# gashon/transformer-lm

Measured on AMD Instinct MI355X. Metric: BPE train input MB/s (32k vocab), train_bpe(path) end to end, higher is better.
Workload: dtype int64

## Files before the change

### transformer-lm_amd/csrc/api.hip

```cpp
#include <dlfcn.h>
#include <hip/hip_version.h>

#include <cerrno>
#include <cstdio>
#include <cstdlib>
#include <cstring>
#include <fstream>
#include <memory>
#include <mutex>
#include <string_view>
#include <unordered_map>
#include <unordered_set>
#include <string>
#include <vector>

#include "count.h"
#include "drive.h"
#include "internal.h"

namespace bpe {

namespace {
thread_local std::string g_err;
thread_local int g_errno = 0;
bool g_timing = false;

struct DeviceGuard {
    static void require() {
        int n = 0;
        if (hipGetDeviceCount(&n) != hipSuccess || n == 0)
            throw Error{BPE_E_HIP, "no HIP device visible (libbpe355 needs an MI355X / gfx950 GPU)"};
    }
};

template <class F>
int guarded(F&& f) {
    try {
        f();
        g_err.clear();
        return BPE_OK;
    } catch (const Error& e) {
        g_err = e.msg;
        g_errno = e.sys_errno;
        return e.code;
    } catch (const std::bad_alloc&) {
        g_err = "host allocation failed";
        return BPE_E_NOMEM;
    } catch (const std::exception& e) {
        g_err = e.what();
        return BPE_E_ARG;
    }
}

std::vector<std::string> to_specials(const char* const* specials, int n) {
    BPE_REQUIRE(n >= 0 && (n == 0 || specials), BPE_E_ARG, "bad special token list");
    std::vector<std::string> v;
    for (int i = 0; i < n; ++i) {
        BPE_REQUIRE(specials[i], BPE_E_ARG, "null special token");
        v.emplace_back(specials[i]);
    }
    return v;
}

struct StreamHolder {
    hipStream_t s = nullptr;
    bool own = false;
    explicit StreamHolder(void* user) {
        if (user) {
            s = (hipStream_t)user;
        } else {
            BPE_HIP(hipStreamCreateWithFlags(&s, hipStreamNonBlocking));
            own = true;
        }
    }
    ~StreamHolder() {
        if (own && s) (void)hipStreamDestroy(s);
    }
};

void put_u32(std::string& b, uint32_t v) { b.append(reinterpret_cast<const char*>(&v), 4); }

}

void set_error(int, const std::string& msg, int sys_errno) {
    g_err = msg;
    g_errno = sys_errno;
}
bool timing_enabled() { return g_timing; }

}

struct bpe_result {
    std::vector<std::pair<std::string, std::string>> merges;
    std::vector<std::string> vocab;
    std::vector<uint32_t> merge_ids;
    int64_t n_merges = 0, n_vocab = 0;
    bpe_train_stats stats{};
    mutable std::once_flag once_mblob, once_vblob, once_flat[2];
    mutable std::string merges_blob, vocab_blob;
    mutable std::vector<uint32_t> flat_len[2];
    mutable std::string flat_bytes[2];
};

struct bpe_comm {
    std::unique_ptr<bpe::Comm> impl;
};

struct bpe_counter {
    mutable std::mutex m;
    bpe::WordAccumulator acc;
};

namespace bpe {
std::unique_ptr<Comm> make_rccl_comm(const uint8_t id[128], int nranks, int rank, int device);
std::unique_ptr<Comm> make_host_comm(bpe_host_allreduce_fn fn, void* ctx, int nranks, int rank,
                                     int device);
}

namespace {

void finish_result(bpe::TrainOutput& out, const std::vector<std::string>& specials, bpe_result* r) {
    const size_t cap = specials.size() + 256 + out.merges.size();
    std::vector<std::string> toks;
    toks.reserve(cap);
    std::unordered_map<std::string_view, uint32_t> id_of;
    id_of.reserve(2 * cap);
    auto add = [&](std::string s) {
        if (id_of.count(s)) return;
        toks.push_back(std::move(s));
        id_of.emplace(toks.back(), (uint32_t)(toks.size() - 1));
    };
    for (const auto& s : specials) add(s);
    for (int b = 0; b < 256; ++b) add(std::string(1, (char)b));
    for (const auto& m : out.merges) add(m.first + m.second);
    r->n_merges = (int64_t)out.merges.size();
    r->n_vocab = (int64_t)toks.size();
    r->merge_ids.reserve(2 * out.merges.size());
    for (const auto& m : out.merges) {
        const auto ia = id_of.find(m.first), ib = id_of.find(m.second);
        if (ia == id_of.end() || ib == id_of.end()) { r->merge_ids.clear(); break; }
        r->merge_ids.push_back(ia->second);
        r->merge_ids.push_back(ib->second);
    }
    id_of.clear();
    r->merges = std::move(out.merges);
    r->vocab = std::move(toks);
    r->stats = out.stats;
}

int train_common(const uint8_t* d_data, size_t n, int vocab_size, const char* const* specials,
                 int n_specials, bpe_comm* comm, void* stream, bpe_result** out) {
    return bpe::guarded([&] {
        BPE_REQUIRE(out, BPE_E_ARG, "out is NULL");
        *out = nullptr;
        bpe::DeviceGuard::require();
        auto sp = bpe::to_specials(specials, n_specials);
        bpe::StreamHolder sh(stream);
        bpe::TrainOutput to;
        bpe::train_on_device(d_data, n, vocab_size, sp, comm ? comm->impl.get() : nullptr, sh.s, to);
        auto r = std::make_unique<bpe_result>();
        finish_result(to, sp, r.get());
        *out = r.release();
    });
}

}

extern "C" {

int bpe_abi_version(void) { return BPE355_ABI_VERSION; }

int bpe_runtime_info(int* compiled_hip_version, int* runtime_hip_version, char* runtime_path, size_t cap) {
    if (compiled_hip_version) *compiled_hip_version = HIP_VERSION;
    int rv = 0;
    const hipError_t e = hipRuntimeGetVersion(&rv);
    if (runtime_hip_version) *runtime_hip_version = e == hipSuccess ? rv : 0;
    if (runtime_path && cap) {
        runtime_path[0] = '\0';
        Dl_info di{};
        if (dladdr(reinterpret_cast<void*>(&hipRuntimeGetVersion), &di) && di.dli_fname)
            std::snprintf(runtime_path, cap, "%s", di.dli_fname);
    }
    return e == hipSuccess ? BPE_OK : BPE_E_HIP;
}
const char* bpe_last_error(void) { return bpe::g_err.c_str(); }
int bpe_last_errno(void) { return bpe::g_errno; }
void bpe_set_timing(int enable) { bpe::g_timing = enable != 0; }

int bpe_release_device_memory(int device, size_t* freed_bytes) {
    return bpe::guarded([&] {
        if (freed_bytes) *freed_bytes = 0;
        int n = 0;
        if (hipGetDeviceCount(&n) != hipSuccess) n = 0;
        BPE_REQUIRE(device < n, BPE_E_ARG, "device " + std::to_string(device) + " is not visible");
        size_t b = bpe::corpus_release(device);
        b += bpe::scratch_release(device);
        if (freed_bytes) *freed_bytes = b;
    });
}

int bpe_device_count(void) {
    int n = 0;
    if (hipGetDeviceCount(&n) != hipSuccess) return 0;
    int k = 0;
    for (int i = 0; i < n; ++i) {
        hipDeviceProp_t p;
        if (hipGetDeviceProperties(&p, i) == hipSuccess && std::strncmp(p.gcnArchName, "gfx950", 6) == 0) ++k;
    }
    return k;
}

int bpe_train_device(const uint8_t* d_data, size_t n, int vocab_size, const char* const* specials,
                     int n_specials, bpe_comm* comm, void* hip_stream, bpe_result** out) {
    if (n && !d_data) return bpe::guarded([] { throw bpe::Error{BPE_E_ARG, "data is NULL"}; });
    return train_common(d_data, n, vocab_size, specials, n_specials, comm, hip_stream, out);
}

int bpe_train_buffer(const uint8_t* data, size_t n, int vocab_size, const char* const* specials,
                     int n_specials, bpe_comm* comm, bpe_result** out) {
    return bpe::guarded([&] {
        BPE_REQUIRE(out, BPE_E_ARG, "out is NULL");
        *out = nullptr;
        BPE_REQUIRE(!n || data, BPE_E_ARG, "data is NULL");
        bpe::DeviceGuard::require();
        auto sp = bpe::to_specials(specials, n_specials);
        const bpe::Source src = bpe::Source::memory(data, n);
        bpe::TrainOutput to;
        if (comm) bpe::train_source_comm(src, false, vocab_size, sp, comm->impl.get(), to);
        else bpe::train_source(src, vocab_size, sp, 1, to);
        auto r = std::make_unique<bpe_result>();
        finish_result(to, sp, r.get());
        *out = r.release();
    });
}

int bpe_train_buffer_gpus(const uint8_t* data, size_t n, int vocab_size, const char* const* specials,
                          int n_specials, int n_gpus, bpe_result** out) {
    return bpe::guarded([&] {
        BPE_REQUIRE(out, BPE_E_ARG, "out is NULL");
        *out = nullptr;
        BPE_REQUIRE(!n || data, BPE_E_ARG, "data is NULL");
        bpe::DeviceGuard::require();
        auto sp = bpe::to_specials(specials, n_specials);
        const bpe::Source src = bpe::Source::memory(data, n);
        bpe::TrainOutput to;
        bpe::train_source(src, vocab_size, sp, n_gpus, to);
        auto r = std::make_unique<bpe_result>();
        finish_result(to, sp, r.get());
        *out = r.release();
    });
}

int bpe_train_file(const char* path, int vocab_size, const char* const* specials, int n_specials,
                   int n_gpus, bpe_result** out) {
    return bpe::guarded([&] {
        BPE_REQUIRE(out, BPE_E_ARG, "out is NULL");
        *out = nullptr;
        BPE_REQUIRE(path, BPE_E_ARG, "path is NULL");
        auto sp = bpe::to_specials(specials, n_specials);
        const bpe::Source src = bpe::Source::open_path(path);
        bpe::DeviceGuard::require();
        bpe::TrainOutput to;
        bpe::train_source(src, vocab_size, sp, n_gpus, to);
        auto r = std::make_unique<bpe_result>();
        finish_result(to, sp, r.get());
        *out = r.release();
    });
}

int bpe_train_file_comm(const char* path, int vocab_size, const char* const* specials, int n_specials,
                        bpe_comm* comm, int split, bpe_result** out) {
    return bpe::guarded([&] {
        BPE_REQUIRE(out, BPE_E_ARG, "out is NULL");
        *out = nullptr;
        BPE_REQUIRE(path, BPE_E_ARG, "path is NULL");
        auto sp = bpe::to_specials(specials, n_specials);
        const bpe::Source src = bpe::Source::open_path(path);
        bpe::DeviceGuard::require();
        bpe::TrainOutput to;
        bpe::train_source_comm(src, split != 0, vocab_size, sp, comm ? comm->impl.get() : nullptr, to);
        auto r = std::make_unique<bpe_result>();
        finish_result(to, sp, r.get());
        *out = r.release();
    });
}

int bpe_word_counts(const uint8_t* data, size_t n, const char* const* specials, int n_specials,
                    uint8_t** blob, size_t* blob_n) {
    return bpe::guarded([&] {
        BPE_REQUIRE(blob && blob_n, BPE_E_ARG, "blob is NULL");
        *blob = nullptr;
        *blob_n = 0;
        BPE_REQUIRE(!n || data, BPE_E_ARG, "data is NULL");
        bpe::DeviceGuard::require();
        auto sp = bpe::to_specials(specials, n_specials);
        bpe::StreamHolder sh(nullptr);
        bpe::DevBuf<uint8_t> d(std::max<size_t>(n, 1)), scratch;
        if (n) BPE_HIP(hipMemcpyAsync(d.p, data, n, hipMemcpyHostToDevice, sh.s));
        size_t tn = 0;
        const uint8_t* text = bpe::prepare_text(d.p, n, scratch, &tn, sh.s);
        bpe::WordCounts wc;
        bpe::count_words(text, tn, wc, sh.s, nullptr);
        std::vector<unsigned long long> kv(2 * wc.cap), pos(wc.cap);
        std::string t(tn, '\0');
        BPE_HIP(hipMemcpyAsync(kv.data(), wc.kv.p, kv.size() * 8, hipMemcpyDeviceToHost, sh.s));
        BPE_HIP(hipMemcpyAsync(pos.data(), wc.pos.p, pos.size() * 8, hipMemcpyDeviceToHost, sh.s));
        if (tn) BPE_HIP(hipMemcpyAsync(&t[0], text, tn, hipMemcpyDeviceToHost, sh.s));
        BPE_HIP(hipStreamSynchronize(sh.s));
        std::unordered_set<std::string> skip(sp.begin(), sp.end());
        std::string out;
        for (size_t i = 0; i < wc.cap; ++i) {
            const unsigned long long k = kv[2 * i];
            if (!k) continue;
            const bool inl = (k >> 63) != 0;
            const size_t len = inl ? (size_t)((k >> 56) & 0x7f) : (size_t)(k >> 40);
            const size_t off = inl ? (size_t)pos[i] : (size_t)((k & ((1ULL << 40) - 1)) - 1);
            const std::string w = t.substr(off, len);
            if (skip.count(w)) continue;
            bpe::put_u32(out, (uint32_t)len);
            out += w;
            const unsigned long long c = kv[2 * i + 1];
            out.append(reinterpret_cast<const char*>(&c), 8);
        }
        *blob = static_cast<uint8_t*>(std::malloc(std::max<size_t>(out.size(), 1)));
        BPE_REQUIRE(*blob, BPE_E_NOMEM, "host allocation failed");
        std::memcpy(*blob, out.data(), out.size());
        *blob_n = out.size();
    });
}

void bpe_blob_free(uint8_t* blob) { std::free(blob); }

int bpe_counter_create(bpe_counter** out) {
    return bpe::guarded([&] {
        BPE_REQUIRE(out, BPE_E_ARG, "out is NULL");
        *out = nullptr;
        bpe::DeviceGuard::require();
        *out = new bpe_counter;
    });
}

int bpe_counter_add_file(bpe_counter* c, const char* path, size_t window_bytes) {
    return bpe::guarded([&] {
        BPE_REQUIRE(c, BPE_E_ARG, "counter is NULL");
        BPE_REQUIRE(path, BPE_E_ARG, "path is NULL");
        const bpe::Source src = bpe::Source::open_path(path);
        std::lock_guard<std::mutex> g(c->m);
        bpe::counter_add_source(c->acc, src, window_bytes);
    });
}

int bpe_counter_add_buffer(bpe_counter* c, const uint8_t* data, size_t n) {
    return bpe::guarded([&] {
        BPE_REQUIRE(c, BPE_E_ARG, "counter is NULL");
        BPE_REQUIRE(!n || data, BPE_E_ARG, "data is NULL");
        const bpe::Source src = bpe::Source::memory(data, n);
        std::lock_guard<std::mutex> g(c->m);
        bpe::counter_add_source(c->acc, src, 0);
    });
}

int bpe_counter_add_device(bpe_counter* c, const uint8_t* d_data, size_t n, void* hip_stream) {
    return bpe::guarded([&] {
        BPE_REQUIRE(c, BPE_E_ARG, "counter is NULL");
        BPE_REQUIRE(!n || d_data, BPE_E_ARG, "data is NULL");
        std::lock_guard<std::mutex> g(c->m);
        bpe::counter_add_device(c->acc, d_data, n, (hipStream_t)hip_stream);
    });
}

int bpe_counter_add_words(bpe_counter* c, const uint8_t* blob, size_t blob_n) {
    return bpe::guarded([&] {
        BPE_REQUIRE(c, BPE_E_ARG, "counter is NULL");
        BPE_REQUIRE(!blob_n || blob, BPE_E_ARG, "blob is NULL");
        std::lock_guard<std::mutex> g(c->m);
        c->acc.add_records(blob, blob_n);
    });
}

int bpe_counter_absorb(bpe_counter* dst, const bpe_counter* src) {
    return bpe::guarded([&] {
        BPE_REQUIRE(dst && src, BPE_E_ARG, "counter is NULL");
        BPE_REQUIRE(dst != src, BPE_E_ARG, "a counter cannot absorb itself");
        std::scoped_lock g(dst->m, src->m);
        dst->acc.absorb(src->acc);
    });
}

int bpe_counter_words(const bpe_counter* c, const char* const* specials, int n_specials, uint8_t** blob,
                      size_t* blob_n) {
    return bpe::guarded([&] {
        BPE_REQUIRE(blob && blob_n, BPE_E_ARG, "blob is NULL");
        *blob = nullptr;
        *blob_n = 0;
        BPE_REQUIRE(c, BPE_E_ARG, "counter is NULL");
        auto sp = bpe::to_specials(specials, n_specials);
        std::lock_guard<std::mutex> g(c->m);
        c->acc.export_words(sp, blob, blob_n);
    });
}

int bpe_counter_train(const bpe_counter* c, int vocab_size, const char* const* specials, int n_specials,
                      bpe_result** out) {
    return bpe::guarded([&] {
        BPE_REQUIRE(out, BPE_E_ARG, "out is NULL");
        *out = nullptr;
        BPE_REQUIRE(c, BPE_E_ARG, "counter is NULL");
        auto sp = bpe::to_specials(specials, n_specials);
        bpe::TrainOutput to;
        {
            std::lock_guard<std::mutex> g(c->m);
            c->acc.train(vocab_size, sp, to);
        }
        auto r = std::make_unique<bpe_result>();
        finish_result(to, sp, r.get());
        *out = r.release();
    });
}

int bpe_counter_info(const bpe_counter* c, bpe_counter_info_t* out) {
    return bpe::guarded([&] {
        BPE_REQUIRE(c && out, BPE_E_ARG, "counter or out is NULL");
        std::lock_guard<std::mutex> g(c->m);
        const bpe::AccumInfo i = c->acc.info();
// ... 118 lines not shown
```

### transformer-lm_amd/csrc/bpe_common.h

```cpp
#pragma once

#include <hip/hip_runtime.h>

#include <cstddef>
#include <cstdint>
#include <string>

#include "../../include/bpe355.h"

namespace bpe {

void set_error(int code, const std::string& msg, int sys_errno = 0);
struct Error {
    int code;
    std::string msg;
    int sys_errno = 0;
};

#define BPE_HIP(expr)                                                                     \
    do {                                                                                  \
        hipError_t e_ = (expr);                                                           \
        if (e_ != hipSuccess)                                                             \
            throw ::bpe::Error{BPE_E_HIP, std::string(#expr) + ": " + hipGetErrorString(e_) + \
                                              " (" __FILE__ ":" + std::to_string(__LINE__) + ")"}; \
    } while (0)

#define BPE_REQUIRE(cond, code, msg)                          \
    do {                                                      \
        if (!(cond)) throw ::bpe::Error{(code), (msg)};       \
    } while (0)

template <class T>
struct DevBuf {
    T* p = nullptr;
    size_t n = 0;
    DevBuf() = default;
    explicit DevBuf(size_t count) { alloc(count); }
    DevBuf(const DevBuf&) = delete;
    DevBuf& operator=(const DevBuf&) = delete;
    DevBuf(DevBuf&& o) noexcept : p(o.p), n(o.n) { o.p = nullptr; o.n = 0; }
    DevBuf& operator=(DevBuf&& o) noexcept {
        if (this != &o) { release(); p = o.p; n = o.n; o.p = nullptr; o.n = 0; }
        return *this;
    }
    ~DevBuf() { release(); }
    void alloc(size_t count) {
        release();
        if (!count) return;
        const hipError_t e = hipMalloc(&p, count * sizeof(T));
        if (e == hipErrorOutOfMemory) {
            (void)hipGetLastError();
            p = nullptr;
            throw ::bpe::Error{BPE_E_NOMEM, "device allocation of " + std::to_string(count * sizeof(T)) +
                                                " bytes failed (out of memory)"};
        }
        BPE_HIP(e);
        n = count;
    }
    void reserve(size_t count) {
        if (count > n || !p) alloc(count);
    }
    void release() {
        if (p) (void)hipFree(p);
        p = nullptr;
        n = 0;
    }
    size_t bytes() const { return n * sizeof(T); }
};

enum : int { CLS_OTHER = 0, CLS_LETTER = 1, CLS_NUMBER = 2, CLS_SPACE = 3 };

__host__ __device__ inline uint64_t mix64(uint64_t z) {
    z ^= z >> 30; z *= 0xBF58476D1CE4E5B9ULL;
    z ^= z >> 27; z *= 0x94D049BB133111EBULL;
    return z ^ (z >> 31);
}

__device__ __forceinline__ unsigned wave_append(bool pred, unsigned* counter) {
    const unsigned long long m = __ballot(pred);
    if (!m) return ~0u;
    const int leader = __ffsll((long long)m) - 1;
    const unsigned lane = threadIdx.x & 63;
    unsigned base = 0;
    if ((int)lane == leader) base = atomicAdd(counter, (unsigned)__popcll(m));
    base = __shfl(base, leader);
    const unsigned below = __builtin_amdgcn_mbcnt_hi((unsigned)(m >> 32),
                                                     __builtin_amdgcn_mbcnt_lo((unsigned)m, 0u));
    return pred ? base + below : ~0u;
}

template <class T>
__device__ __forceinline__ T wave_sum(T v) {
    for (int o = 32; o > 0; o >>= 1) v += __shfl_xor(v, o);
    return v;
}

template <class T>
__device__ __forceinline__ T wave_max(T v) {
    for (int o = 32; o > 0; o >>= 1) {
        const T w = __shfl_xor(v, o);
        v = w > v ? w : v;
    }
    return v;
}

inline unsigned ceil_div(size_t a, size_t b) { return (unsigned)((a + b - 1) / b); }
constexpr size_t kMaxGridBlocks = 1u << 20;
inline unsigned grid_for(size_t items, unsigned block) {
    const size_t b = (items + block - 1) / block;
    return (unsigned)(b < kMaxGridBlocks ? (b ? b : 1) : kMaxGridBlocks);
}
inline size_t next_pow2(size_t x) {
    size_t p = 1;
    while (p < x) p <<= 1;
    return p;
}

}
```

### transformer-lm_amd/csrc/comm.hip

```cpp
#include <rccl/rccl.h>

#include <algorithm>
#include <condition_variable>
#include <cstring>
#include <mutex>
#include <memory>
#include <vector>

#include "internal.h"

namespace bpe {

namespace {

#define BPE_NCCL(expr)                                                                       \
    do {                                                                                     \
        ncclResult_t r_ = (expr);                                                            \
        if (r_ != ncclSuccess)                                                               \
            throw Error{BPE_E_RCCL, std::string(#expr) + ": " + ncclGetErrorString(r_)};     \
    } while (0)

struct RcclComm final : Comm {
    ncclComm_t comm = nullptr;
    RcclComm(const uint8_t id[128], int n, int r, int dev) {
        nranks = n;
        rank = r;
        device = dev;
        BPE_HIP(hipSetDevice(dev));
        ncclUniqueId uid;
        static_assert(sizeof(uid.internal) == 128, "ncclUniqueId size");
        std::memcpy(uid.internal, id, 128);
        BPE_NCCL(ncclCommInitRank(&comm, n, uid, r));
    }
    ~RcclComm() override {
        if (comm) (void)ncclCommDestroy(comm);
    }
    void allreduce_i64(int64_t* d_buf, size_t count, hipStream_t stream) override {
        if (count == 0) return;
        BPE_NCCL(ncclAllReduce(d_buf, d_buf, count, ncclInt64, ncclSum, comm, stream));
    }
    void allgather_bytes(const void* d_send, size_t bytes, void* d_recv, hipStream_t stream) override {
        if (bytes == 0) return;
        BPE_NCCL(ncclAllGather(d_send, d_recv, bytes, ncclUint8, comm, stream));
    }
    void alltoallv_bytes(const void* d_send, const size_t* soff, const size_t* scnt, void* d_recv,
                         const size_t* roff, const size_t* rcnt, hipStream_t stream) override {
        const uint8_t* snd = static_cast<const uint8_t*>(d_send);
        uint8_t* rcv = static_cast<uint8_t*>(d_recv);
        if (scnt[rank])
            BPE_HIP(hipMemcpyAsync(rcv + roff[rank], snd + soff[rank], scnt[rank], hipMemcpyDeviceToDevice, stream));
        BPE_NCCL(ncclGroupStart());
        for (int p = 0; p < nranks; ++p) {
            if (p == rank) continue;
            if (scnt[p]) BPE_NCCL(ncclSend(snd + soff[p], scnt[p], ncclUint8, p, comm, stream));
            if (rcnt[p]) BPE_NCCL(ncclRecv(rcv + roff[p], rcnt[p], ncclUint8, p, comm, stream));
        }
        BPE_NCCL(ncclGroupEnd());
    }
};

struct HostComm final : Comm {
    bpe_host_allreduce_fn fn;
    void* ctx;
    std::vector<int64_t> buf;
    HostComm(bpe_host_allreduce_fn f, void* c, int n, int r, int dev) : fn(f), ctx(c) {
        nranks = n;
        rank = r;
        device = dev;
    }
    void allreduce_i64(int64_t* d_buf, size_t count, hipStream_t stream) override {
        if (count == 0) return;
        buf.resize(count);
        BPE_HIP(hipMemcpyAsync(buf.data(), d_buf, count * 8, hipMemcpyDeviceToHost, stream));
        BPE_HIP(hipStreamSynchronize(stream));
        BPE_REQUIRE(fn(ctx, buf.data(), count) == 0, BPE_E_RCCL, "host all-reduce callback failed");
        BPE_HIP(hipMemcpyAsync(d_buf, buf.data(), count * 8, hipMemcpyHostToDevice, stream));
        BPE_HIP(hipStreamSynchronize(stream));
    }
};

struct InProcShared {
    std::mutex m;
    std::condition_variable cv;
    int arrived = 0;
    uint64_t gen = 0;
    std::vector<int64_t> acc, result;
    std::vector<uint8_t> gather;
    int g_entered = 0, g_readers = 0;
    std::vector<std::vector<uint8_t>> a2a;
    std::vector<std::vector<size_t>> a2a_off, a2a_cnt;
    bool failed = false;
};

struct InProcComm final : Comm {
    std::shared_ptr<InProcShared> sh;
    std::vector<int64_t> h;
    InProcComm(std::shared_ptr<InProcShared> s, int n, int r, int dev) : sh(std::move(s)) {
        nranks = n;
        rank = r;
        device = dev;
    }
    template <class Op>
    void guarded(const Op& op) {
        try {
            op();
        } catch (...) {
            {
                std::lock_guard<std::mutex> g(sh->m);
                sh->failed = true;
            }
            sh->cv.notify_all();
            throw;
        }
    }
    void check_failed() const {
        BPE_REQUIRE(!sh->failed, BPE_E_RCCL, "in-process collective: another rank failed");
    }
    void allreduce_i64(int64_t* d_buf, size_t count, hipStream_t stream) override {
        if (count == 0) return;
        guarded([&] {
            h.resize(count);
            BPE_HIP(hipMemcpyAsync(h.data(), d_buf, count * 8, hipMemcpyDeviceToHost, stream));
            BPE_HIP(hipStreamSynchronize(stream));
            {
                std::unique_lock<std::mutex> lk(sh->m);
                check_failed();
                const uint64_t g = sh->gen;
                if (sh->arrived == 0) sh->acc.assign(count, 0);
                BPE_REQUIRE(sh->acc.size() == count, BPE_E_RCCL, "in-process all-reduce: ranks disagree on the size");
                for (size_t i = 0; i < count; ++i) sh->acc[i] += h[i];
                if (++sh->arrived == nranks) {
                    sh->result.swap(sh->acc);
                    sh->arrived = 0;
                    ++sh->gen;
                    sh->cv.notify_all();
                } else {
                    sh->cv.wait(lk, [&] { return sh->gen != g || sh->failed; });
                    check_failed();
                }
                h = sh->result;
            }
            BPE_HIP(hipMemcpyAsync(d_buf, h.data(), count * 8, hipMemcpyHostToDevice, stream));
            BPE_HIP(hipStreamSynchronize(stream));
        });
    }
    void allgather_bytes(const void* d_send, size_t bytes, void* d_recv, hipStream_t stream) override {
        if (bytes == 0) return;
        guarded([&] {
            std::unique_lock<std::mutex> lk(sh->m);
            sh->cv.wait(lk, [&] { return sh->g_readers == 0 || sh->failed; });
            check_failed();
            const uint64_t g = sh->gen;
            if (sh->g_entered == 0) sh->gather.assign((size_t)nranks * bytes, 0);
            BPE_REQUIRE(sh->gather.size() == (size_t)nranks * bytes, BPE_E_RCCL,
                        "in-process all-gather: ranks disagree on the size");
            ++sh->g_entered;
            uint8_t* mine = sh->gather.data() + (size_t)rank * bytes;
            lk.unlock();
            BPE_HIP(hipMemcpyAsync(mine, d_send, bytes, hipMemcpyDeviceToHost, stream));
            BPE_HIP(hipStreamSynchronize(stream));
            lk.lock();
            check_failed();
// ... 98 lines not shown
```

### transformer-lm_amd/csrc/count.hip

```cpp
#include <hip/hip_ext.h>

#include <algorithm>
#include <cstdlib>
#include <mutex>
#include <vector>

#include "count.h"
#include "pretok.h"
#include "prims.h"
#include "stage.h"
#include "stage2.h"
#include "tokstart.h"

#ifndef BPE355_COUNT_EARLY_PREFETCH
#define BPE355_COUNT_EARLY_PREFETCH 1
#endif

namespace bpe {

namespace {

constexpr int kCache2 = 512;
constexpr int kEpoch2 = 4;
constexpr unsigned kKeep2 = 2;
constexpr unsigned kCntBits = 19;
constexpr unsigned kRecReserve = kChunk / 2 + 1 + 2 * kCache2;
constexpr int kBinBits = 12;
constexpr int kBins = 1 << kBinBits;

__device__ __forceinline__ unsigned rec_bin(uint64_t h) { return (unsigned)(h >> (64 - kBinBits)); }

template <bool kAligned>
__global__ void __launch_bounds__(256) __attribute__((amdgpu_waves_per_eu(4))) k_count2(const uint8_t* __restrict__ s, size_t lo, size_t n, size_t chunk0,
                                                size_t n_chunks, unsigned long long* __restrict__ kv,
                                                unsigned long long* __restrict__ pos, size_t mask,
                                                unsigned long long max_fill, unsigned long long* __restrict__ fill,
                                                unsigned* __restrict__ status, unsigned long long* __restrict__ n_tok,
                                                RecPool R, const unsigned long long* __restrict__ gate, int mode) {
    if (gate && *gate != ~0ULL) return;
    __shared__ uint64_t s_mask[kWords];
    __shared__ unsigned long long c_key[kCache2];
    __shared__ uint64_t c_lo[kCache2], c_hi[kCache2];
    __shared__ unsigned c_cnt[kCache2];
    __shared__ uint16_t c_mark[kCache2];
    __shared__ unsigned long long s_red[4];
    __shared__ int s_stop, s_page, s_old;
    __shared__ unsigned s_used;
    __shared__ unsigned s_ch[kCoarse];
    __shared__ unsigned s_nlong;
    const int tid = threadIdx.x;
    for (int i = tid; i < kCache2; i += blockDim.x) { c_key[i] = 0; c_cnt[i] = 0; c_mark[i] = 0; }
    load_cls2(tid, blockDim.x);
    if (tid == 0) {
        s_page = R.on ? R.wg_page[blockIdx.x] : -1;
        s_used = R.on ? R.wg_used[blockIdx.x] : 0u;
        s_nlong = R.lw ? R.lw_n[blockIdx.x] : 0u;
    }
    if (tid < kCoarse) s_ch[tid] = R.on ? R.wg_ch[(size_t)blockIdx.x * kCoarse + tid] : 0u;
    unsigned long long ntok = 0, inserted = 0, n_miss = 0, n_long = 0;

    auto spill = [&](uint64_t wl, uint64_t wh, size_t len, size_t gpos, unsigned long long c, uint64_t h) {
        const int pg = s_page;
        if (pg >= 0 && c < (1ULL << kCntBits)) {
            atomicAdd(&s_ch[h >> (64 - kCoarseBits)], 1u);
            const unsigned idx = atomicAdd(&s_used, 1u);
            const size_t gi = (size_t)pg * kPageRecs + idx;
            R.lo[gi] = wl;
            R.hi[gi] = wh;
            R.meta[gi] = (unsigned long long)len | ((unsigned long long)gpos << 5) | (c << 45);
            return;
        }
        bool ins;
        table_add(s, s, gpos, len, wl, wh, h, c, kv, pos, mask, status, &ins);
        inserted += ins;
    };

    uint4 pre[kSVec];
    if (blockIdx.x < n_chunks) fetch2<kAligned>(pre, s, n, (chunk0 + blockIdx.x) * kChunk, tid);
    for (size_t c = blockIdx.x; c < n_chunks; c += gridDim.x) {
        __syncthreads();
        store2(pre, tid);
        if (tid == 0) {
            s_stop = *(volatile unsigned long long*)fill > max_fill;
            s_old = -3;
            if (R.on && s_page != -1 && (s_page == -2 || s_used + kRecReserve > (unsigned)kPageRecs)) {
                if (s_page >= 0) R.page_used[s_page] = s_used;
                s_old = s_page;
                const unsigned pg = atomicAdd(R.n_pages, 1u);
                s_page = pg < R.max_pages ? (int)pg : -1;
                s_used = 0;
            }
        }
        __syncthreads();
        if (s_old != -3 && tid < kCoarse) {
            if (s_old >= 0) R.page_ch[(size_t)s_old * kCoarse + tid] = s_ch[tid];
            s_ch[tid] = 0;
        }
        if (s_stop) {
            if (tid == 0) atomicOr(status, 1u);
            break;
        }
        const size_t base = (chunk0 + c) * kChunk;
        if (BPE355_COUNT_EARLY_PREFETCH && c + gridDim.x < n_chunks)
            fetch2<kAligned>(pre, s, n, (chunk0 + c + gridDim.x) * kChunk, tid);

        auto mask_word = [&](int w) -> uint64_t {
            const int r0 = kPre + 64 * w - kStartPre;
            const size_t blk = base + 64 * (size_t)w;
            const long long vhi = (long long)n - ((long long)blk - kStartPre);
            uint64_t m = token_starts64<DevTab>(LdsWin{r0}, (int)(vhi < kStartWin ? (vhi > 0 ? vhi : 0) : kStartWin));
            if (blk + 64 <= lo) {
                m = 0;
            } else if (blk <= lo) {
                const int k = (int)(lo - blk);
                m = (m & (~0ULL << k)) | (1ULL << k);
            }
            return m;
        };
        s_mask[tid] = mask_word(tid);
        if (!BPE355_COUNT_EARLY_PREFETCH && c + gridDim.x < n_chunks)
            fetch2<kAligned>(pre, s, n, (chunk0 + c + gridDim.x) * kChunk, tid);
        __syncthreads();

        if (mode == 1) continue;
        const size_t rem = n > base ? n - base : 0;
        const uint32_t tend = rem < (size_t)kWin ? (uint32_t)rem : (uint32_t)kWin;
        uint64_t m = s_mask[tid];
        while (m) {
            const uint32_t r = 64u * tid + (uint32_t)__builtin_ctzll(m);
            m &= m - 1;
            size_t e;
            if (m) {
                e = 64u * tid + (uint32_t)__builtin_ctzll(m);
            } else {
                e = ~(size_t)0;
                for (int w = tid + 1; w < kWords; ++w) {
                    const uint64_t x = s_mask[w];
                    if (x) { e = 64u * w + (uint32_t)__builtin_ctzll(x); break; }
                }
                if (e == ~(size_t)0) {
                    e = token_end(StageText{}, tend, r);
                    if (e + 4 > tend && tend < rem) e = token_end(s, n, base + r) - base;
                }
            }
            const size_t len = e - r;
            if (len < 2) continue;
            ++ntok;
            if (mode == 2) continue;
            const size_t gpos = base + r;
            if (len > (size_t)kInline) {
                ++n_long;
                if (mode == 5) continue;
                if (R.lw && len < kMaxPretok) {
                    const unsigned li = atomicAdd(&s_nlong, 1u);
                    if (li < R.lw_per_wg) {
                        R.lw[(size_t)blockIdx.x * R.lw_per_wg + li] = (unsigned long long)gpos | ((unsigned long long)len << 40);
                        continue;
                    }
                }
                bool ins;
                table_add(s, s, gpos, len, 0, 0, hash_word(s, gpos, len), 1, kv, pos, mask, status, &ins);
                inserted += ins;
                continue;
            }
            uint64_t wl, wh;
// ... 475 lines not shown
        if (k == 0) continue;
        const size_t len = (size_t)(k >> 40), off = (size_t)(k & kOffMask) - 1;
        const uint64_t wl = t_lo[i], wh = t_hi[i];
        bool ins;
        table_add(s, s, off, len, wl, wh, short_hash(wl, wh, len), t_cnt[i], kv, pos, mask, status, &ins);
        inserted += ins;
    }
    inserted = wave_sum(inserted);
    if ((threadIdx.x & 63) == 0 && inserted) atomicAdd(fill, inserted);
}

int count2_per_cu() {
    static int per_cu = 0;
    if (!per_cu)
        BPE_HIP(hipOccupancyMaxActiveBlocksPerMultiprocessor(&per_cu, k_count2<true>, 256, kStage));
    return std::max(per_cu, 1);
}

}

unsigned count2_grid(size_t n_chunks) {
    static int n_cu = 0;
    if (!n_cu) {
        int dev = 0;
        BPE_HIP(hipGetDevice(&dev));
        BPE_HIP(hipDeviceGetAttribute(&n_cu, hipDeviceAttributeMultiprocessorCount, dev));
    }
    (void)n_chunks;
    unsigned grid = (unsigned)count2_per_cu() * (unsigned)std::max(1, n_cu);
    if (const char* e = std::getenv("BPE355_STREAM_WG"))
        grid = std::max(1u, std::min(grid, (unsigned)std::atoi(e)));
    return grid;
}

void count2_launch(const uint8_t* text, size_t lo, size_t hi, size_t c0, size_t nc, unsigned grid,
                   const WordCounts& wc, unsigned long long* fill, unsigned* status, unsigned long long* ntok,
                   const RecPool& R, const unsigned long long* gate, hipStream_t s, hipEvent_t e0, hipEvent_t e1) {
    static const int mode = std::getenv("BPE355_COUNT_MODE") ? std::atoi(std::getenv("BPE355_COUNT_MODE")) : 0;
    const bool aligned = (reinterpret_cast<uintptr_t>(text) & 15u) == 0;
    auto kern = aligned ? k_count2<true> : k_count2<false>;
    hipExtLaunchKernelGGL(kern, dim3(grid), dim3(256), kStage, s, e0, e1, 0, text, lo, hi, c0, nc, wc.kv.p, wc.pos.p,
                          wc.cap - 1, (unsigned long long)(wc.cap / 2), fill, status, ntok, R, gate, mode);
    BPE_HIP(hipGetLastError());
}

void count_long_launch(const uint8_t* text, const WordCounts& wc, unsigned long long* fill, unsigned* status,
                       const RecPool& R, unsigned grid, hipStream_t s) {
    if (!R.lw) return;
    hipLaunchKernelGGL(k_count_long, dim3(grid), dim3(256), 0, s, text, R, wc.kv.p, wc.pos.p, wc.cap - 1, fill, status);
    BPE_HIP(hipGetLastError());
}

namespace {
struct ScratchArrays {
    std::mutex m;
    std::vector<std::unique_ptr<Arrays3>> free_;
};
ScratchArrays& scratch() {
    static ScratchArrays* p = new ScratchArrays;
    return *p;
}
}

std::unique_ptr<Arrays3> scratch_take(size_t cap) {
    int dev = 0;
    BPE_HIP(hipGetDevice(&dev));
    std::unique_ptr<Arrays3> x;
    {
        std::lock_guard<std::mutex> g(scratch().m);
        auto& f = scratch().free_;
        size_t best = f.size();
        for (size_t i = 0; i < f.size(); ++i)
            if (f[i]->dev == dev && f[i]->cap >= cap && (best == f.size() || f[i]->cap < f[best]->cap)) best = i;
        if (best == f.size())
            for (size_t i = 0; i < f.size(); ++i)
                if (f[i]->dev == dev && (best == f.size() || f[i]->cap > f[best]->cap)) best = i;
        if (best < f.size()) {
            x = std::move(f[best]);
            f.erase(f.begin() + best);
        }
    }
    if (x && x->cap >= cap) return x;
    x.reset();
    x = std::make_unique<Arrays3>();
    x->dev = dev;
    x->cap = cap;
    try {
        x->a.alloc(cap);
        x->b.alloc(cap);
        x->c.alloc(cap);
    } catch (const Error& e) {
        if (e.code != BPE_E_NOMEM) throw;
        x->a.release(); x->b.release(); x->c.release(); x->d.release();
        scratch_release(dev);
        x->a.alloc(cap);
        x->b.alloc(cap);
        x->c.alloc(cap);
    }
    return x;
}

size_t scratch_cached_bytes(int dev) {
    std::lock_guard<std::mutex> g(scratch().m);
    size_t b = 0;
    for (auto& f : scratch().free_)
        if (f->dev == dev) b += f->bytes();
    return b;
}

size_t scratch_release(int dev) {
    std::vector<std::unique_ptr<Arrays3>> drop;
    size_t bytes = 0;
    {
        std::lock_guard<std::mutex> g(scratch().m);
        auto& f = scratch().free_;
        for (size_t i = 0; i < f.size();)
            if (dev < 0 || f[i]->dev == dev) {
                bytes += f[i]->bytes();
                drop.push_back(std::move(f[i]));
                f.erase(f.begin() + i);
            } else {
                ++i;
            }
    }
    if (drop.empty()) return bytes;
    int cur = 0;
    BPE_HIP(hipGetDevice(&cur));
    for (auto& x : drop) {
        (void)hipSetDevice(x->dev);
        x.reset();
    }
    BPE_HIP(hipSetDevice(cur));
    return bytes;
}

void scratch_give(std::unique_ptr<Arrays3> x) {
    if (!x) return;
    std::lock_guard<std::mutex> g(scratch().m);
    scratch().free_.push_back(std::move(x));
}

RecPoolOwner::~RecPoolOwner() {
    scratch_give(std::move(rec));
    scratch_give(std::move(B));
}

void RecPoolOwner::init(size_t n_bytes, unsigned grid, hipStream_t s) {
    size_t want = std::max<size_t>(n_bytes / 10, (size_t)grid * kPageRecs);
    if (const char* e = std::getenv("BPE355_REC_POOL")) want = (size_t)std::atof(e);
    int dev = 0;
    BPE_HIP(hipGetDevice(&dev));
    size_t free_b = 0, total_b = 0;
    BPE_HIP(hipMemGetInfo(&free_b, &total_b));
    const size_t avail = free_b + scratch_cached_bytes(dev);
    const size_t reserve = std::max<size_t>(total_b / 16, n_bytes / 2);
    size_t fit = avail > reserve ? (avail - reserve) / (6 * sizeof(uint64_t) + 1) : 0;
    if (const char* e = std::getenv("BPE355_REC_POOL_FIT")) fit = (size_t)std::atof(e);
    if (fit < want) {
        if (fit < (size_t)grid * kPageRecs / 4)
            throw Error{BPE_E_NOMEM, "record pool: " + std::to_string(avail) + " bytes of device memory free"};
        want = fit;
    }
    max_pages = (unsigned)std::max<size_t>(1, std::min<size_t>((want + kPageRecs - 1) / kPageRecs, 1u << 30));
    const size_t cap = (size_t)max_pages * kPageRecs;
    if (std::getenv("BPE355_REC_POOL_FAIL"))
        throw Error{BPE_E_NOMEM, "record pool allocation failed (BPE355_REC_POOL_FAIL)"};
    rec = scratch_take(cap);
    page_used.alloc(max_pages);
    page_ch.alloc((size_t)max_pages * kCoarse);
    n_pages.alloc(1);
    wg_page.alloc(grid);
    wg_used.alloc(grid);
    wg_ch.alloc((size_t)grid * kCoarse);
    BPE_HIP(hipMemsetAsync(wg_ch.p, 0, 4ull * grid * kCoarse, s));
    held.alloc(max_pages);
    done.alloc(max_pages);
    lw_per_wg = (unsigned)std::min<size_t>(1u << 24, std::max<size_t>(1024, n_bytes / 1024 / grid + 1));
    if (const char* e = std::getenv("BPE355_LONG_SEG")) lw_per_wg = (unsigned)std::max(1, std::atoi(e));
    lw.alloc((size_t)lw_per_wg * grid);
    lw_n.alloc(grid);
    BPE_HIP(hipMemsetAsync(lw_n.p, 0, 4ull * grid, s));
    B = scratch_take(cap);
    if (B->d.n < cap) B->d.alloc(cap);
    max_tiles = max_pages + kCoarse;
    coff.alloc((size_t)kCoarse * max_pages);
    ctot.alloc(kCoarse);
    cbase.alloc(kCoarse + 1);
    d_tl.alloc(max_tiles);
    d_t0.alloc(kCoarse + 1);
    fhist.alloc((size_t)kCoarse * max_tiles);
    ftot.alloc(kBins);
    fbase.alloc(kBins + 1);
    n_tiles.alloc(1);
    d_records.alloc(1);
    BPE_HIP(hipMemsetAsync(d_records.p, 0, 8, s));
    list.alloc(max_pages);
    list_n.alloc(1);
    BPE_HIP(hipMemsetAsync(held.p, 0, 4ull * max_pages, s));
    BPE_HIP(hipMemsetAsync(done.p, 0, 4ull * max_pages, s));
    n_wg = grid;
    BPE_HIP(hipMemsetAsync(n_pages.p, 0, 4, s));
    BPE_HIP(hipMemsetAsync(wg_used.p, 0, 4ull * grid, s));
    std::vector<int> none(grid, -2);
    BPE_HIP(hipMemcpyAsync(wg_page.p, none.data(), 4ull * grid, hipMemcpyHostToDevice, s));
    BPE_HIP(hipStreamSynchronize(s));
}

RecPool RecPoolOwner::dev() const {
    RecPool R{};
    R.lo = rec ? rec->a.p : nullptr;
    R.hi = rec ? rec->b.p : nullptr;
    R.meta = rec ? rec->c.p : nullptr;
    R.page_used = page_used.p;
    R.n_pages = n_pages.p;
    R.max_pages = max_pages;
    R.wg_page = wg_page.p;
    R.wg_used = wg_used.p;
    R.page_ch = page_ch.p;
    R.wg_ch = wg_ch.p;
    R.lw = lw.p;
    R.lw_n = lw_n.p;
    R.lw_per_wg = lw_per_wg;
    R.on = rec != nullptr;
    return R;
}

void RecPoolOwner::aggregate(bool final, const uint8_t* text, const WordCounts& wc, unsigned long long* fill,
                             unsigned* status, hipStream_t s) {
    const RecPool R = dev();
    if (final) {
        hipLaunchKernelGGL(k_rec_retire, dim3(ceil_div(n_wg, 256)), dim3(256), 0, s, R, n_wg);
    } else {
        hipLaunchKernelGGL(k_rec_hold, dim3(ceil_div(n_wg, 256)), dim3(256), 0, s, R, n_wg, held.p);
    }
    BPE_HIP(hipMemsetAsync(list_n.p, 0, 4, s));
    hipLaunchKernelGGL(k_rec_pick, dim3(ceil_div(max_pages, 256)), dim3(256), 0, s, R, held.p, done.p, list.p,
                       list_n.p);
    ++batches;
    hipLaunchKernelGGL(k_rec_cscan, dim3(kCoarse), dim3(1024), 0, s, page_ch.p, list.p, list_n.p, coff.p, ctot.p);
    hipLaunchKernelGGL(k_rec_tiles, dim3(1), dim3(64), 0, s, ctot.p, cbase.p, d_tl.p, d_t0.p, n_tiles.p,
                       d_records.p);
    hipLaunchKernelGGL(k_rec_part1, dim3(max_pages), dim3(1024), 0, s, R, list.p, list_n.p, coff.p, cbase.p, B->a.p,
                       B->b.p, B->c.p, B->d.p);
    hipLaunchKernelGGL(k_rec_fhist, dim3(max_tiles), dim3(1024), 0, s, B->d.p, d_tl.p, n_tiles.p, fhist.p);
    hipLaunchKernelGGL(k_rec_fscan, dim3(kBins), dim3(256), 0, s, fhist.p, d_t0.p, ftot.p);
    hipLaunchKernelGGL(k_rec_base, dim3(1), dim3(1024), 0, s, ftot.p, kBins, fbase.p);
    hipLaunchKernelGGL(k_rec_part2, dim3(max_tiles), dim3(1024), 0, s, B->a.p, B->b.p, B->c.p, d_tl.p, n_tiles.p,
                       fhist.p, fbase.p, R.lo, R.hi, R.meta, list.p);
    hipLaunchKernelGGL(k_rec_reduce, dim3(kBins), dim3(1024), 0, s, R.lo, R.hi, R.meta, fbase.p, list.p, text,
                       wc.kv.p, wc.pos.p, wc.cap - 1, fill, status);
    BPE_HIP(hipGetLastError());
    if (final) {
        unsigned long long tot = 0;
        unsigned allocated = 0;
        BPE_HIP(hipMemcpyAsync(&tot, d_records.p, 8, hipMemcpyDeviceToHost, s));
        BPE_HIP(hipMemcpyAsync(&allocated, n_pages.p, 4, hipMemcpyDeviceToHost, s));
        BPE_HIP(hipStreamSynchronize(s));
        records = tot;
        pages_used = std::min(allocated, max_pages);
    }
}

}
```

### transformer-lm_amd/csrc/drive.hip

```cpp
#include <fcntl.h>
#include <sys/stat.h>
#include <unistd.h>

#include <rccl/rccl.h>

#include <algorithm>
#include <atomic>
#include <condition_variable>
#include <cerrno>
#include <chrono>
#include <cstdio>
#include <cstring>
#include <exception>
#include <memory>
#include <mutex>
#include <thread>
#include <vector>

#include "drive.h"

namespace bpe {

namespace {

constexpr size_t kStageChunk = 16u << 20;

struct PinnedPool {
    std::mutex m;
    std::vector<void*> free_;
    void* get() {
        {
            std::lock_guard<std::mutex> g(m);
            if (!free_.empty()) {
                void* p = free_.back();
                free_.pop_back();
                return p;
            }
        }
        void* p = nullptr;
        BPE_HIP(hipHostMalloc(&p, kStageChunk, hipHostMallocPortable));
        return p;
    }
    void put(void* p) {
        std::lock_guard<std::mutex> g(m);
        free_.push_back(p);
    }
};
PinnedPool& pool() {
    static PinnedPool* p = new PinnedPool;
    return *p;
}

struct MappedBuf {
    void* host = nullptr;
    void* dev = nullptr;
};
struct MappedPool {
    std::mutex m;
    std::vector<MappedBuf> free_;
    MappedBuf get() {
        {
            std::lock_guard<std::mutex> g(m);
            if (!free_.empty()) {
                const MappedBuf b = free_.back();
                free_.pop_back();
                return b;
            }
        }
        MappedBuf b;
        BPE_HIP(hipHostMalloc(&b.host, kStageChunk, hipHostMallocMapped | hipHostMallocCoherent | hipHostMallocPortable));
        const hipError_t e = hipHostGetDevicePointer(&b.dev, b.host, 0);
        if (e != hipSuccess) {
            (void)hipHostFree(b.host);
            BPE_HIP(e);
        }
        return b;
    }
    void put(const MappedBuf& b) {
        std::lock_guard<std::mutex> g(m);
        free_.push_back(b);
    }
};
MappedPool& mapped_pool() {
    static MappedPool* p = new MappedPool;
    return *p;
}

__global__ void __launch_bounds__(256) k_to_host(const uint8_t* __restrict__ src, uint8_t* __restrict__ dst, size_t n) {
    const size_t stride = (size_t)gridDim.x * blockDim.x;
    const size_t t = (size_t)blockIdx.x * blockDim.x + threadIdx.x;
    if ((((uintptr_t)src | (uintptr_t)dst) & 15u) == 0) {
        const size_t n16 = n / 16;
        for (size_t i = t; i < n16; i += stride)
            reinterpret_cast<uint4*>(dst)[i] = reinterpret_cast<const uint4*>(src)[i];
        for (size_t i = n16 * 16 + t; i < n; i += stride) dst[i] = src[i];
    } else {
        for (size_t i = t; i < n; i += stride) dst[i] = src[i];
    }
}
int d2h_wg() {
    int n = 0;
    if (const char* e = std::getenv("BPE355_D2H_WG")) n = std::atoi(e);
    return std::max(0, std::min(n, 1024));
}

struct CorpusBuf {
    DevBuf<uint8_t> b;
    int dev = -1;
};
struct CorpusCache {
    std::mutex m;
    std::vector<std::unique_ptr<CorpusBuf>> free_;
};
CorpusCache& corpus_cache() {
    static CorpusCache* c = new CorpusCache;
    return *c;
}
std::unique_ptr<CorpusBuf> corpus_take(size_t n) {
    int dev = 0;
    BPE_HIP(hipGetDevice(&dev));
    std::unique_ptr<CorpusBuf> x;
    {
        std::lock_guard<std::mutex> g(corpus_cache().m);
        auto& f = corpus_cache().free_;
        for (size_t i = 0; i < f.size(); ++i)
            if (f[i]->dev == dev) {
                x = std::move(f[i]);
                f.erase(f.begin() + i);
                break;
            }
    }
    if (x && x->b.n >= n) return x;
    if (!x) x = std::make_unique<CorpusBuf>();
    x->b.release();
    x->b.alloc(n);
    x->dev = dev;
    return x;
}
void corpus_give(std::unique_ptr<CorpusBuf> x) {
    std::lock_guard<std::mutex> g(corpus_cache().m);
    corpus_cache().free_.push_back(std::move(x));
}

[[noreturn]] void io_error(int en, const std::string& what) {
    throw Error{BPE_E_IO, what + ": " + std::strerror(en), en};
}

}

size_t corpus_release(int dev) {
    std::vector<std::unique_ptr<CorpusBuf>> drop;
    size_t bytes = 0;
    {
        std::lock_guard<std::mutex> g(corpus_cache().m);
        auto& f = corpus_cache().free_;
        for (size_t i = 0; i < f.size();)
            if (dev < 0 || f[i]->dev == dev) {
                bytes += f[i]->b.bytes();
                drop.push_back(std::move(f[i]));
                f.erase(f.begin() + i);
            } else {
                ++i;
            }
    }
    if (drop.empty()) return bytes;
    int cur = 0;
    BPE_HIP(hipGetDevice(&cur));
    for (auto& x : drop) {
        (void)hipSetDevice(x->dev);
        x->b.release();
    }
    BPE_HIP(hipSetDevice(cur));
// ... 129 lines not shown
        if (r == 0) io_error(EIO, "short read on " + name + " (file truncated while reading?)");
        got += (size_t)r;
    }
}

std::vector<size_t> slab_cuts(const Source& src, int g) {
    std::vector<size_t> cut(g + 1, 0);
    cut[g] = src.size;
    std::vector<uint8_t> win;
    for (int r = 1; r < g; ++r) {
        const size_t want = src.size / g * r;
        size_t c = cut[r - 1];
        for (size_t w = 1u << 16; w <= (64u << 20); w <<= 2) {
            const size_t lo = want > w ? want - w : 0;
            const size_t hi = std::min(src.size, want + 2);
            if (hi <= lo + 2) break;
            win.resize(hi - lo);
            src.read(lo, hi - lo, win.data());
            const size_t p = bpe_safe_split(win.data(), win.size(), want - lo);
            if (p > 0 && lo + p > cut[r - 1]) { c = lo + p; break; }
            if (lo == 0) break;
        }
        cut[r] = c;
    }
    return cut;
}

void stage_to_device(const Source& src, size_t off, size_t len, uint8_t* d_dst, int device, int threads) {
    if (len == 0) return;
    const size_t chunks = (len + kStageChunk - 1) / kStageChunk;
    const int t_n = (int)std::max<size_t>(1, std::min<size_t>((size_t)threads, chunks));
    std::atomic<size_t> next{0};
    std::vector<std::exception_ptr> errs(t_n);
    const DmaStreams& dma = cached_dma(device, 0);
    auto work = [&](int t) {
        const hipStream_t s = dma.pick(t);
        void* buf[2] = {nullptr, nullptr};
        hipEvent_t ev[2] = {nullptr, nullptr};
        bool busy[2] = {false, false};
        try {
            BPE_HIP(hipSetDevice(device));
            for (int k = 0; k < 2; ++k) {
                buf[k] = pool().get();
                BPE_HIP(hipEventCreateWithFlags(&ev[k], hipEventDisableTiming));
            }
            for (int k = 0;; k ^= 1) {
                const size_t i = next.fetch_add(1);
                if (i >= chunks) break;
                if (busy[k]) BPE_HIP(hipEventSynchronize(ev[k]));
                const size_t lo = i * kStageChunk, n = std::min(kStageChunk, len - lo);
                src.read(off + lo, n, static_cast<uint8_t*>(buf[k]));
                BPE_HIP(hipMemcpyAsync(d_dst + lo, buf[k], n, hipMemcpyHostToDevice, s));
                BPE_HIP(hipEventRecord(ev[k], s));
                busy[k] = true;
            }
        } catch (...) {
            errs[t] = std::current_exception();
            next.store(chunks);
            (void)hipStreamSynchronize(s);
        }
        for (int k = 0; k < 2; ++k) {
            if (busy[k]) (void)hipEventSynchronize(ev[k]);
            if (ev[k]) (void)hipEventDestroy(ev[k]);
            if (buf[k]) pool().put(buf[k]);
        }
    };
    std::vector<std::thread> th;
    for (int t = 1; t < t_n; ++t) th.emplace_back(work, t);
    work(0);
    for (auto& x : th) x.join();
    for (auto& e : errs)
        if (e) std::rethrow_exception(e);
}

void device_to_host(const uint8_t* d_src, size_t len, uint8_t* h_dst, int device, int threads) {
    if (len == 0) return;
    const size_t chunks = (len + kStageChunk - 1) / kStageChunk;
    const int t_n = (int)std::max<size_t>(1, std::min<size_t>((size_t)threads, chunks));
    std::atomic<size_t> next{0};
    std::vector<std::exception_ptr> errs(t_n);
    const DmaStreams& dma = cached_dma(device, 1);
    auto work = [&](int t) {
        const hipStream_t s = dma.pick(t);
        const int wg = d2h_wg();
        void* buf[2] = {nullptr, nullptr};
        MappedBuf mb[2];
        hipEvent_t ev[2] = {nullptr, nullptr};
        size_t pend[2] = {~(size_t)0, ~(size_t)0};
        auto drain = [&](int k) {
            if (pend[k] == ~(size_t)0) return;
            BPE_HIP(hipEventSynchronize(ev[k]));
            const size_t lo = pend[k] * kStageChunk;
            std::memcpy(h_dst + lo, buf[k], std::min(kStageChunk, len - lo));
            pend[k] = ~(size_t)0;
        };
        try {
            BPE_HIP(hipSetDevice(device));
            for (int k = 0; k < 2; ++k) {
                if (wg) {
                    mb[k] = mapped_pool().get();
                    buf[k] = mb[k].host;
                } else {
                    buf[k] = pool().get();
                }
                BPE_HIP(hipEventCreateWithFlags(&ev[k], hipEventDisableTiming));
            }
            for (int k = 0;; k ^= 1) {
                drain(k);
                const size_t i = next.fetch_add(1);
                if (i >= chunks) break;
                const size_t lo = i * kStageChunk, n = std::min(kStageChunk, len - lo);
                if (wg) {
                    hipLaunchKernelGGL(k_to_host, dim3(wg), dim3(256), 0, s, d_src + lo, static_cast<uint8_t*>(mb[k].dev), n);
                    BPE_HIP(hipGetLastError());
                } else {
                    BPE_HIP(hipMemcpyAsync(buf[k], d_src + lo, n, hipMemcpyDeviceToHost, s));
                }
                BPE_HIP(hipEventRecord(ev[k], s));
                pend[k] = i;
            }
            drain(0);
            drain(1);
        } catch (...) {
            errs[t] = std::current_exception();
            next.store(chunks);
            (void)hipStreamSynchronize(s);
        }
        for (int k = 0; k < 2; ++k) {
            if (pend[k] != ~(size_t)0) (void)hipEventSynchronize(ev[k]);
            if (ev[k]) (void)hipEventDestroy(ev[k]);
            if (buf[k]) {
                if (wg) mapped_pool().put(mb[k]);
                else pool().put(buf[k]);
            }
        }
    };
    std::vector<std::thread> th;
    for (int t = 1; t < t_n; ++t) th.emplace_back(work, t);
    work(0);
    for (auto& x : th) x.join();
    for (auto& e : errs)
        if (e) std::rethrow_exception(e);
}

namespace {

struct ChunkTrack {
    std::vector<hipEvent_t> ev;
    std::vector<char> ready;
    std::mutex m;
    std::condition_variable cv;
    size_t prefix = 0;
    bool failed = false;
    explicit ChunkTrack(size_t n) : ev(n, nullptr), ready(n, 0) {
        for (auto& e : ev) BPE_HIP(hipEventCreateWithFlags(&e, hipEventDisableTiming));
    }
    ~ChunkTrack() {
        for (auto& e : ev)
            if (e) (void)hipEventDestroy(e);
    }
    void mark(size_t i) {
        std::lock_guard<std::mutex> g(m);
        ready[i] = 1;
        while (prefix < ready.size() && ready[prefix]) ++prefix;
        cv.notify_all();
    }
    void fail() {
        std::lock_guard<std::mutex> g(m);
        failed = true;
        cv.notify_all();
    }
    bool wait_prefix(size_t k) {
        std::unique_lock<std::mutex> lk(m);
        cv.wait(lk, [&] { return prefix >= k || failed; });
        return !failed;
    }
};

size_t segment_bytes() {
    const char* e = std::getenv("BPE355_SEG_MB");
    return (size_t)(e ? std::max(1, std::atoi(e)) : 256) << 20;
}

std::vector<size_t> segment_cuts(const Source& src, size_t off, size_t len, size_t seg) {
    std::vector<size_t> cut{0};
    std::vector<uint8_t> win(1u << 16);
    for (size_t want = seg; want + seg / 2 < len; want += seg) {
        const size_t lo = want - std::min(want, win.size() - 2);
        const size_t hi = want + 2;
        src.read(off + lo, hi - lo, win.data());
        const size_t p = bpe_safe_split(win.data(), hi - lo, want - lo);
        if (p > 0 && lo + p > cut.back()) cut.push_back(lo + p);
    }
    cut.push_back(len);
    return cut;
}

}

bool load_and_count(const Source& src, size_t off, size_t len, uint8_t* d_dst, int device, int threads,
                    hipStream_t stream, Prepared& pre, size_t min_cap) {
    const auto t0 = std::chrono::steady_clock::now();
    const std::vector<size_t> cut = segment_cuts(src, off, len, segment_bytes());
    const size_t chunks = (len + kStageChunk - 1) / kStageChunk;
    ChunkTrack track(chunks);
    const int t_n = (int)std::max<size_t>(1, std::min<size_t>((size_t)threads, chunks));
    std::atomic<size_t> next{0};
    std::vector<std::exception_ptr> errs(t_n);
    DmaStreams dma(device, dma_streams());
    auto reader = [&](int t) {
        const hipStream_t s = dma.pick(t);
        void* buf[2] = {nullptr, nullptr};
        size_t last[2] = {~(size_t)0, ~(size_t)0};
        try {
            BPE_HIP(hipSetDevice(device));
            for (int k = 0; k < 2; ++k) buf[k] = pool().get();
            for (int k = 0;; k ^= 1) {
                const size_t i = next.fetch_add(1);
                if (i >= chunks) break;
                if (last[k] != ~(size_t)0) BPE_HIP(hipEventSynchronize(track.ev[last[k]]));
                const size_t lo = i * kStageChunk, n = std::min(kStageChunk, len - lo);
                src.read(off + lo, n, static_cast<uint8_t*>(buf[k]));
                BPE_HIP(hipMemcpyAsync(d_dst + lo, buf[k], n, hipMemcpyHostToDevice, s));
                BPE_HIP(hipEventRecord(track.ev[i], s));
                last[k] = i;
                track.mark(i);
            }
        } catch (...) {
            errs[t] = std::current_exception();
            next.store(chunks);
            track.fail();
            (void)hipStreamSynchronize(s);
        }
        for (int k = 0; k < 2; ++k) {
            if (last[k] != ~(size_t)0) (void)hipEventSynchronize(track.ev[last[k]]);
            if (buf[k]) pool().put(buf[k]);
        }
    };
    std::vector<std::thread> th;
    for (int t = 0; t < t_n; ++t) th.emplace_back(reader, t);
    ValidatePass vp;
    CountPass cp;
    bool ok = true;
    const char* ae = std::getenv("BPE355_AGG_SEGS");
    const size_t agg_every = ae ? (size_t)std::max(0, std::atoi(ae)) : 4;
    try {
        vp.begin(d_dst, len, stream);
        cp.begin(d_dst, len, std::max(CountPass::initial_cap(len), min_cap), stream, timing_enabled());
        cp.gate = vp.flags.p;
        size_t waited = 0;
        for (size_t k = 0; k + 1 < cut.size(); ++k) {
            const size_t need = (cut[k + 1] + kStageChunk - 1) / kStageChunk;
            if (!track.wait_prefix(need)) { ok = false; break; }
            for (; waited < need; ++waited) BPE_HIP(hipStreamWaitEvent(stream, track.ev[waited], 0));
            vp.range(cut[k], cut[k + 1]);
            cp.range(cut[k], cut[k + 1]);
            if (agg_every > 0 && (k + 1) % agg_every == 0 && k + 2 < cut.size()) cp.partial();
        }
    } catch (...) {
        track.fail();
        next.store(chunks);
        for (auto& x : th) x.join();
        throw;
    }
    for (auto& x : th) x.join();
    for (auto& e : errs)
        if (e) std::rethrow_exception(e);
    BPE_REQUIRE(ok, BPE_E_IO, "corpus load failed");
    const double load_ms = std::chrono::duration<double, std::milli>(std::chrono::steady_clock::now() - t0).count();
    unsigned long long bad = 0;
    bool cr = false;
    vp.finish(&bad, &cr);
    if (bad != ~0ULL)
        throw Error{BPE_E_UTF8, "'utf-8' codec can't decode byte at position " + std::to_string(bad)};
    if (cr) return false;
    if (!cp.finish()) {
        float kms = 0;
        count_words(d_dst, len, cp.wc, stream, timing_enabled() ? &kms : nullptr);
        cp.kernel_ms += kms;
    }
    pre.text = d_dst;
    pre.n = len;
    pre.wc = std::move(cp.wc);
    pre.count_kernel_ms = (float)cp.kernel_ms;
    pre.t_prepare_ms = 0;
    pre.t_count_ms = std::chrono::duration<double, std::milli>(std::chrono::steady_clock::now() - t0).count() - load_ms;
    pre.load_ms = load_ms;
    return true;
}

namespace {

size_t next_safe_split(const Source& src, size_t from) {
    auto ascii_nonspace = [](uint8_t b) { return b < 0x80 && b != 0x20 && (b < 0x09 || b > 0x0D); };
    std::vector<uint8_t> win((1u << 16) + 2);
    for (size_t p = std::max<size_t>(from, 1); p + 1 < src.size;) {
        const size_t lo = p - 1, hi = std::min(src.size, lo + win.size());
        src.read(lo, hi - lo, win.data());
        for (size_t i = 1; i + 1 < hi - lo; ++i)
            if (win[i] == 0x20 && ascii_nonspace(win[i - 1]) && ascii_nonspace(win[i + 1])) return lo + i;
        p = hi - 1;
    }
    return src.size;
}

std::vector<size_t> window_cuts(const Source& src, size_t window) {
    std::vector<size_t> cut{0};
    std::vector<uint8_t> win((1u << 16) + 2);
    while (src.size - cut.back() > window) {
        const size_t start = cut.back(), want = start + window;
        const size_t lo = std::max(start, want - (win.size() - 2)), hi = std::min(src.size, want + 2);
        src.read(lo, hi - lo, win.data());
        const size_t p = bpe_safe_split(win.data(), hi - lo, want - lo);
        size_t end = p > 0 && lo + p > start ? lo + p : next_safe_split(src, want);
        if (end >= src.size) break;
        cut.push_back(end);
    }
    cut.push_back(src.size);
    return cut;
}

size_t window_table_slots(const WordAccumulator& a, const WordAccumulator& b, size_t len) {
    const size_t seen = std::max(a.shard_words_hint(), b.shard_words_hint());
    return next_pow2(std::max<size_t>(len / 128, 4 * seen));
}

[[noreturn]] void rethrow_at(const Error& e, size_t offset) {
    Error err = e;
    const size_t p = err.msg.find("position ");
    if (err.code == BPE_E_UTF8 && offset && p != std::string::npos)
        err.msg = "'utf-8' codec can't decode byte at position " +
                  std::to_string(std::stoull(err.msg.substr(p + 9)) + offset);
    throw err;
}

}

void counter_add_source(WordAccumulator& acc, const Source& src, size_t window_bytes) {
    const size_t window = std::max<size_t>(window_bytes ? window_bytes : kDefaultWindow, (size_t)64 << 10);
    int cur = 0;
    BPE_HIP(hipGetDevice(&cur));
    const int dev = acc.device();
    struct DevGuard { int prev; ~DevGuard() { (void)hipSetDevice(prev); } } dg{cur};
    BPE_HIP(hipSetDevice(dev));
    const std::vector<size_t> cut = window_cuts(src, window);
    const size_t n_win = cut.size() - 1;
    size_t max_win = 0;
    for (size_t k = 0; k < n_win; ++k) max_win = std::max(max_win, cut[k + 1] - cut[k]);
    std::unique_ptr<WordAccumulator> tmp;
    if (n_win > 1) tmp = std::make_unique<WordAccumulator>();
    WordAccumulator& into = tmp ? *tmp : acc;
    const hipStream_t s = into.stream();
    std::unique_ptr<CorpusBuf> d = corpus_take(std::max<size_t>(max_win, 1));
    struct Give { std::unique_ptr<CorpusBuf>& d; ~Give() { if (d) corpus_give(std::move(d)); } } give{d};
    double load_ms = 0, count_ms = 0;
    uint64_t n_bytes = 0;
    for (size_t k = 0; k < n_win; ++k) {
        const size_t off = cut[k], len = cut[k + 1] - off;
        Prepared pre;
        DevBuf<uint8_t> scratch;
        const uint8_t* text = d->b.p;
        size_t tn = len;
        WordCounts wc;
        try {
            const auto t0 = std::chrono::steady_clock::now();
            if (load_and_count(src, off, len, d->b.p, dev, io_threads(), s, pre, window_table_slots(into, acc, len))) {
                wc = std::move(pre.wc);
                load_ms += pre.load_ms;
                count_ms += pre.t_count_ms;
            } else {
                const double loaded = std::chrono::duration<double, std::milli>(std::chrono::steady_clock::now() - t0).count();
                text = prepare_text(d->b.p, len, scratch, &tn, s);
                count_words(text, tn, wc, s, nullptr);
                load_ms += loaded;
                count_ms += std::chrono::duration<double, std::milli>(std::chrono::steady_clock::now() - t0).count() - loaded;
            }
        } catch (const Error& e) {
            (void)hipStreamSynchronize(s);
            rethrow_at(e, off);
        }
        BPE_HIP(hipStreamSynchronize(s));
        into.fold(text, wc, tn);
        n_bytes += tn;
    }
    into.note_input(n_bytes, n_win, max_win, load_ms, count_ms);
    if (tmp) acc.absorb(*tmp);
}

void counter_add_device(WordAccumulator& acc, const uint8_t* d_data, size_t n, hipStream_t stream) {
    int cur = 0;
    BPE_HIP(hipGetDevice(&cur));
    struct DevGuard { int prev; ~DevGuard() { (void)hipSetDevice(prev); } } dg{cur};
    BPE_HIP(hipSetDevice(acc.device()));
    const hipStream_t s = stream ? stream : acc.stream();
    const auto t0 = std::chrono::steady_clock::now();
    DevBuf<uint8_t> scratch;
    size_t tn = 0;
    const uint8_t* text = prepare_text(d_data, n, scratch, &tn, s);
    WordCounts wc;
    count_words(text, tn, wc, s, nullptr);
    BPE_HIP(hipStreamSynchronize(s));
    const double count_ms = std::chrono::duration<double, std::milli>(std::chrono::steady_clock::now() - t0).count();
    acc.fold(text, wc, tn);
    acc.note_input(tn, 1, n, 0, count_ms);
}

bool inproc_ranks() { return std::getenv("BPE355_INPROC_RANKS") != nullptr; }

std::vector<int> pick_devices(int n_gpus) {
    int cur = 0, n = 0;
    BPE_HIP(hipGetDevice(&cur));
    BPE_HIP(hipGetDeviceCount(&n));
    BPE_REQUIRE(n > 0, BPE_E_HIP, "no HIP device visible");
    const int want = n_gpus <= 0 ? n : n_gpus;
    BPE_REQUIRE(want <= n || inproc_ranks(), BPE_E_ARG,
                "n_gpus = " + std::to_string(n_gpus) + " but only " + std::to_string(n) + " devices are visible");
    std::vector<int> d;
    for (int i = 0; i < want; ++i) d.push_back((cur + i) % n);
    return d;
}

void train_source(const Source& src, int vocab_size, const std::vector<std::string>& specials, int n_gpus,
                  TrainOutput& out) {
    const auto t0 = std::chrono::steady_clock::now();
    const std::vector<int> dev = pick_devices(n_gpus);
    const int g = (int)dev.size();
    if (g == 1) {
        static const bool dtrace = std::getenv("BPE355_DRIVE_TRACE") != nullptr;
        auto ms = [&] { return std::chrono::duration<double, std::milli>(std::chrono::steady_clock::now() - t0).count(); };
        hipStream_t s = nullptr;
        BPE_HIP(hipStreamCreateWithFlags(&s, hipStreamNonBlocking));
        struct SGuard { hipStream_t s; ~SGuard() { (void)hipStreamDestroy(s); } } sg{s};
        std::unique_ptr<CorpusBuf> d = corpus_take(std::max<size_t>(src.size, 1));
        const double a_ms = ms();
        Prepared pre;
        const bool counted = load_and_count(src, 0, src.size, d->b.p, dev[0], io_threads(), s, pre);
        const double load_ms = counted ? a_ms + pre.load_ms : ms();
        const double before_train = ms();
        train_on_device(d->b.p, src.size, vocab_size, specials, nullptr, s, out, TrainOpts{}, counted ? &pre : nullptr);
        if (dtrace) {
            const double tr = ms();
            std::fprintf(stderr, "[bpe355 drive] alloc %.1f stage %.1f train %.1f ms\n", a_ms, load_ms - a_ms,
                         tr - load_ms);
        }
        corpus_give(std::move(d));
        out.stats.t_load_ms = load_ms;
        out.stats.t_total_ms += before_train;
        out.stats.n_gpus = 1;
        return;
    }
    const std::vector<size_t> cut = slab_cuts(src, g);
    const bool inproc = inproc_ranks();
    uint8_t id[128] = {};
    std::shared_ptr<void> group;
    if (inproc) group = make_inproc_group();
    else BPE_REQUIRE(bpe_comm_unique_id(id) == BPE_OK, BPE_E_RCCL, "ncclGetUniqueId failed");
    std::vector<TrainOutput> outs(g);
    std::vector<std::exception_ptr> errs(g);
    std::vector<double> load_ms(g, 0);
    const int per = std::max(2, io_threads() / g);
    auto work = [&](int r) {
        try {
            BPE_HIP(hipSetDevice(dev[r]));
            hipStream_t s = nullptr;
            BPE_HIP(hipStreamCreateWithFlags(&s, hipStreamNonBlocking));
            struct SGuard { hipStream_t s; ~SGuard() { (void)hipStreamDestroy(s); } } sg{s};
            const size_t len = cut[r + 1] - cut[r];
            std::unique_ptr<CorpusBuf> dbuf = corpus_take(std::max<size_t>(len, 1));
            uint8_t* const d = dbuf->b.p;
            TrainOpts opt;
            opt.slab_offset = cut[r];
            opt.merge_loop = r == 0 || per_round_exchange();
            Prepared pre;
            bool counted = false;
            try {
                counted = load_and_count(src, cut[r], len, d, dev[r], per, s, pre);
            } catch (const Error& e) {
                opt.pending = e;
                opt.has_pending = true;
            }
            load_ms[r] = std::chrono::duration<double, std::milli>(std::chrono::steady_clock::now() - t0).count();
            auto comm = inproc ? make_inproc_comm(group, g, r, dev[r]) : make_rccl_comm(id, g, r, dev[r]);
            train_on_device(d, len, vocab_size, specials, comm.get(), s, outs[r], opt, counted ? &pre : nullptr);
            BPE_HIP(hipStreamSynchronize(s));
            corpus_give(std::move(dbuf));
        } catch (...) {
            errs[r] = std::current_exception();
        }
    };
    std::vector<std::thread> th;
    for (int r = 1; r < g; ++r) th.emplace_back(work, r);
    work(0);
    for (auto& x : th) x.join();
    for (auto& e : errs)
        if (e) std::rethrow_exception(e);
    if (per_round_exchange())
        for (int r = 1; r < g; ++r)
            BPE_REQUIRE(outs[r].merges == outs[0].merges, BPE_E_RCCL,
                        "rank " + std::to_string(r) + " chose different merges than rank 0");
    out = std::move(outs[0]);
    out.stats.t_load_ms = *std::max_element(load_ms.begin(), load_ms.end());
    out.stats.t_total_ms = std::chrono::duration<double, std::milli>(std::chrono::steady_clock::now() - t0).count();
    out.stats.n_gpus = g;
    int64_t nb = 0;
    for (auto& o : outs) nb += o.stats.n_bytes;
    out.stats.n_bytes = nb;
}

void train_source_comm(const Source& src, bool split, int vocab_size, const std::vector<std::string>& specials,
                       Comm* comm, TrainOutput& out) {
    const auto t0 = std::chrono::steady_clock::now();
    int dev = 0;
    BPE_HIP(hipGetDevice(&dev));
    size_t lo = 0, hi = src.size;
    if (split && comm && comm->nranks > 1) {
        const std::vector<size_t> cut = slab_cuts(src, comm->nranks);
        lo = cut[comm->rank];
        hi = cut[comm->rank + 1];
    }
    hipStream_t s = nullptr;
    BPE_HIP(hipStreamCreateWithFlags(&s, hipStreamNonBlocking));
    struct SGuard { hipStream_t s; ~SGuard() { (void)hipStreamDestroy(s); } } sg{s};
    std::unique_ptr<CorpusBuf> dbuf = corpus_take(std::max<size_t>(hi - lo, 1));
    uint8_t* const d = dbuf->b.p;
    TrainOpts opt;
    opt.slab_offset = lo;
    Prepared pre;
    bool counted = false;
    try {
        counted = load_and_count(src, lo, hi - lo, d, dev, io_threads(), s, pre);
    } catch (const Error& e) {
        if (!comm || comm->nranks == 1) throw;
        opt.pending = e;
        opt.has_pending = true;
    }
    const double before_train = std::chrono::duration<double, std::milli>(std::chrono::steady_clock::now() - t0).count();
    train_on_device(d, hi - lo, vocab_size, specials, comm, s, out, opt, counted ? &pre : nullptr);
    corpus_give(std::move(dbuf));
    out.stats.t_load_ms = counted ? pre.load_ms : before_train;
    out.stats.t_total_ms += before_train;
    out.stats.n_gpus = comm ? comm->nranks : 1;
}

}
```

### transformer-lm_amd/csrc/exchange.hip

```cpp

#include <algorithm>
#include <cstdio>
#include <cstdlib>
#include <vector>

#include <chrono>

#include "internal.h"
#include "prims.h"
#include "stage.h"

namespace bpe {

namespace {

__global__ void k_local_words(const unsigned long long* __restrict__ kv, const unsigned long long* __restrict__ pos,
                              size_t cap, unsigned long long* __restrict__ w_off, uint32_t* __restrict__ w_len,
                              unsigned long long* __restrict__ w_cnt, unsigned* __restrict__ n_words) {
    const size_t s = (size_t)blockIdx.x * blockDim.x + threadIdx.x;
    const unsigned long long k = s < cap ? kv[2 * s] : 0ULL;
    const bool keep = k != 0;
    const bool inl = (k >> 63) != 0;
    const unsigned idx = wave_append(keep, n_words);
    if (!keep) return;
    w_len[idx] = inl ? (unsigned)((k >> 56) & 0x7f) : (unsigned)(k >> 40);
    w_off[idx] = inl ? pos[s] : (k & kOffMask) - 1;
    w_cnt[idx] = kv[2 * s + 1];
}

__global__ void k_len_to_u64(const uint32_t* __restrict__ w_len, unsigned n, unsigned long long* __restrict__ o) {
    const unsigned i = blockIdx.x * blockDim.x + threadIdx.x;
    if (i < n) o[i] = w_len[i];
}

__global__ void k_pack_words(const uint8_t* __restrict__ text, const unsigned long long* __restrict__ w_off,
                             const uint32_t* __restrict__ w_len, const unsigned long long* __restrict__ w_cnt,
                             const unsigned long long* __restrict__ b_off, unsigned n, size_t maxw,
                             uint8_t* __restrict__ seg) {
    const unsigned i = blockIdx.x * blockDim.x + threadIdx.x;
    if (i >= n) return;
    unsigned long long* cnt = reinterpret_cast<unsigned long long*>(seg);
    unsigned long long* lo = cnt + maxw;
    uint8_t* bytes = reinterpret_cast<uint8_t*>(lo + maxw);
    const uint32_t len = w_len[i];
    const unsigned long long o = b_off[i];
    cnt[i] = w_cnt[i];
    lo[i] = ((unsigned long long)len << 32) | o;
    const uint8_t* src = text + w_off[i];
    for (uint32_t k = 0; k < len; ++k) bytes[o + k] = src[k];
}

__global__ void k_union_insert(const uint8_t* __restrict__ all, size_t seg_bytes, size_t maxw,
                               const unsigned long long* __restrict__ nw_per_rank, int nranks,
                               unsigned long long* __restrict__ kv, unsigned long long* __restrict__ pos,
                               size_t mask, unsigned* __restrict__ status) {
    const size_t g = (size_t)blockIdx.x * blockDim.x + threadIdx.x;
    const size_t r = g / maxw, i = g % maxw;
    if ((int)r >= nranks || i >= nw_per_rank[r]) return;
    const uint8_t* seg = all + r * seg_bytes;
    const unsigned long long* cnt = reinterpret_cast<const unsigned long long*>(seg);
    const unsigned long long* lo = cnt + maxw;
    const size_t byte_base = r * seg_bytes + 16 * maxw;
    const unsigned long long c = cnt[i], x = lo[i];
    const size_t len = (size_t)(x >> 32), p = byte_base + (x & 0xffffffffULL);
    uint64_t wl = 0, wh = 0, h;
    if (len <= (size_t)kInline) {
        pack_word(all, p, len, wl, wh);
        h = short_hash(wl, wh, len);
    } else {
        h = hash_word(all, p, len);
    }
    bool ins;
    (void)table_add(all, all, p, len, wl, wh, h, c, kv, pos, mask, status, &ins);
}

constexpr unsigned kMaxOwners = 256;

__device__ __forceinline__ uint64_t word_hash_at(const uint8_t* __restrict__ t, size_t p, size_t len, uint64_t& wl,
                                                 uint64_t& wh) {
    wl = 0;
    wh = 0;
    if (len <= (size_t)kInline) {
        pack_word(t, p, len, wl, wh);
        return short_hash(wl, wh, len);
    }
    return hash_word(t, p, len);
}
__device__ __forceinline__ unsigned owner_of(uint64_t h, unsigned R) { return (unsigned)(((h >> 40) * R) >> 24); }

__global__ void __launch_bounds__(256) k_own_count(const uint8_t* __restrict__ text,
                                                   const unsigned long long* __restrict__ w_off,
                                                   const uint32_t* __restrict__ w_len, unsigned n, unsigned R,
                                                   unsigned* __restrict__ owner, unsigned long long* __restrict__ tot) {
    __shared__ unsigned h_rec[kMaxOwners], h_b[kMaxOwners];
    for (unsigned q = threadIdx.x; q < R; q += blockDim.x) { h_rec[q] = 0; h_b[q] = 0; }
    __syncthreads();
    const unsigned i = blockIdx.x * blockDim.x + threadIdx.x;
    if (i < n) {
        uint64_t wl, wh;
        const uint32_t len = w_len[i];
        const unsigned o = owner_of(word_hash_at(text, w_off[i], len, wl, wh), R);
        owner[i] = o;
        atomicAdd(&h_rec[o], 1u);
        atomicAdd(&h_b[o], len);
    }
    __syncthreads();
    for (unsigned q = threadIdx.x; q < R; q += blockDim.x)
        if (h_rec[q]) {
            atomicAdd(&tot[q], (unsigned long long)h_rec[q]);
            atomicAdd(&tot[R + q], (unsigned long long)h_b[q]);
        }
}

__global__ void __launch_bounds__(256) k_own_place(const uint8_t* __restrict__ text,
                                                   const unsigned long long* __restrict__ w_off,
                                                   const uint32_t* __restrict__ w_len,
                                                   const unsigned long long* __restrict__ w_cnt,
                                                   const unsigned* __restrict__ owner, unsigned n, unsigned R,
                                                   const unsigned long long* __restrict__ seg_off,
                                                   const unsigned long long* __restrict__ seg_nrec,
                                                   unsigned long long* __restrict__ cur, uint8_t* __restrict__ send) {
    __shared__ unsigned l_rec[kMaxOwners], l_b[kMaxOwners];
    __shared__ unsigned long long b_rec[kMaxOwners], b_b[kMaxOwners];
    for (unsigned q = threadIdx.x; q < R; q += blockDim.x) { l_rec[q] = 0; l_b[q] = 0; }
    __syncthreads();
    const unsigned i = blockIdx.x * blockDim.x + threadIdx.x;
    unsigned o = 0, r_loc = 0, b_loc = 0, len = 0;
    if (i < n) {
        o = owner[i];
        len = w_len[i];
        r_loc = atomicAdd(&l_rec[o], 1u);
        b_loc = atomicAdd(&l_b[o], len);
    }
    __syncthreads();
    for (unsigned q = threadIdx.x; q < R; q += blockDim.x)
        if (l_rec[q]) {
            b_rec[q] = atomicAdd(&cur[q], (unsigned long long)l_rec[q]);
            b_b[q] = atomicAdd(&cur[R + q], (unsigned long long)l_b[q]);
        }
    __syncthreads();
    if (i >= n) return;
    const unsigned long long nrec = seg_nrec[o];
    uint8_t* seg = send + seg_off[o];
    unsigned long long* cnt = reinterpret_cast<unsigned long long*>(seg);
    unsigned long long* lo = cnt + nrec;
    uint8_t* bytes = reinterpret_cast<uint8_t*>(lo + nrec);
    const unsigned long long ri = b_rec[o] + r_loc, bo = b_b[o] + b_loc;
    cnt[ri] = w_cnt[i];
    lo[ri] = ((unsigned long long)len << 32) | bo;
    const uint8_t* src = text + w_off[i];
    for (uint32_t k = 0; k < len; ++k) bytes[bo + k] = src[k];
}

__global__ void k_seg_insert(const uint8_t* __restrict__ buf, const unsigned long long* __restrict__ seg_off,
                             const unsigned long long* __restrict__ seg_nrec,
                             const unsigned long long* __restrict__ seg_stride, int nseg, size_t maxw,
                             unsigned long long* __restrict__ kv, unsigned long long* __restrict__ pos, size_t mask,
                             unsigned* __restrict__ status) {
    const size_t g = (size_t)blockIdx.x * blockDim.x + threadIdx.x;
    const size_t r = g / maxw, i = g % maxw;
    if ((int)r >= nseg || i >= seg_nrec[r]) return;
    const unsigned long long* cnt = reinterpret_cast<const unsigned long long*>(buf + seg_off[r]);
    const unsigned long long* lo = cnt + seg_stride[r];
// ... 279 lines not shown
```

### transformer-lm_amd/csrc/hostio.hip

```cpp
#include <algorithm>
#include <cstring>

#include "internal.h"

namespace bpe {
namespace {

constexpr size_t kMailbox = 8u << 20;

__global__ void k_blit(const uint8_t* __restrict__ src, uint8_t* __restrict__ dst, size_t n) {
    const size_t stride = (size_t)gridDim.x * blockDim.x;
    const size_t t = (size_t)blockIdx.x * blockDim.x + threadIdx.x;
    if ((((uintptr_t)src | (uintptr_t)dst) & 15u) == 0) {
        const size_t n16 = n / 16;
        for (size_t i = t; i < n16; i += stride)
            reinterpret_cast<uint4*>(dst)[i] = reinterpret_cast<const uint4*>(src)[i];
        for (size_t i = n16 * 16 + t; i < n; i += stride) dst[i] = src[i];
    } else {
        for (size_t i = t; i < n; i += stride) dst[i] = src[i];
    }
}

struct Mailbox {
    uint8_t* host = nullptr;
    uint8_t* dev = nullptr;
    Mailbox() {
        BPE_HIP(hipHostMalloc(reinterpret_cast<void**>(&host), kMailbox,
                              hipHostMallocMapped | hipHostMallocCoherent | hipHostMallocPortable));
        BPE_HIP(hipHostGetDevicePointer(reinterpret_cast<void**>(&dev), host, 0));
    }
    ~Mailbox() {
        if (host) (void)hipHostFree(host);
    }
};
Mailbox& mailbox() {
    thread_local Mailbox m;
    return m;
}

void blit(const uint8_t* src, uint8_t* dst, size_t n, hipStream_t s) {
    const unsigned blocks = (unsigned)std::min<size_t>(1024, std::max<size_t>(1, (n / 16 + 255) / 256));
    hipLaunchKernelGGL(k_blit, dim3(blocks), dim3(256), 0, s, src, dst, n);
    BPE_HIP(hipGetLastError());
}

}

void to_host(void* dst, const void* d_src, size_t bytes, hipStream_t s) {
    Mailbox& m = mailbox();
    for (size_t off = 0; off < bytes; off += kMailbox) {
        const size_t k = std::min(kMailbox, bytes - off);
        blit(static_cast<const uint8_t*>(d_src) + off, m.dev, k, s);
        BPE_HIP(hipStreamSynchronize(s));
        std::memcpy(static_cast<uint8_t*>(dst) + off, m.host, k);
    }
}

void to_device(void* d_dst, const void* src, size_t bytes, hipStream_t s) {
    Mailbox& m = mailbox();
    for (size_t off = 0; off < bytes; off += kMailbox) {
        const size_t k = std::min(kMailbox, bytes - off);
        std::memcpy(m.host, static_cast<const uint8_t*>(src) + off, k);
        blit(m.dev, static_cast<uint8_t*>(d_dst) + off, k, s);
        BPE_HIP(hipStreamSynchronize(s));
    }
}

}
```

### transformer-lm_amd/csrc/text.hip

```cpp

#include <cstdio>
#include <cstdlib>

#include <hip/hip_ext.h>

#include "count.h"
#include "internal.h"
#include "prims.h"
#include "pretok.h"
#include "stage.h"

namespace bpe {

__device__ __forceinline__ int utf8_len_valid(const uint8_t* __restrict__ s, size_t n, size_t i) {
    const uint32_t b0 = s[i];
    uint32_t need, lo = 0x80, hi = 0xBF;
    if (b0 < 0x80u) return 1;
    if (b0 >= 0xC2u && b0 <= 0xDFu) need = 2;
    else if (b0 == 0xE0u) { need = 3; lo = 0xA0; }
    else if (b0 >= 0xE1u && b0 <= 0xECu) need = 3;
    else if (b0 == 0xEDu) { need = 3; hi = 0x9F; }
    else if (b0 >= 0xEEu && b0 <= 0xEFu) need = 3;
    else if (b0 == 0xF0u) { need = 4; lo = 0x90; }
    else if (b0 >= 0xF1u && b0 <= 0xF3u) need = 4;
    else if (b0 == 0xF4u) { need = 4; hi = 0x8F; }
    else return 0;
    if (i + need > n) return 0;
    const uint32_t b1 = s[i + 1];
    if (b1 < lo || b1 > hi) return 0;
    for (uint32_t k = 2; k < need; ++k)
        if ((s[i + k] & 0xC0u) != 0x80u) return 0;
    return (int)need;
}

__device__ __forceinline__ bool byte_ok(const uint8_t* __restrict__ s, size_t n, size_t i) {
    const uint32_t b = s[i];
    if (b < 0x80u) return true;
    if ((b & 0xC0u) != 0x80u) return utf8_len_valid(s, n, i) > 0;
    size_t q = i;
    for (int k = 0; k < 3 && q > 0; ++k) {
        --q;
        if ((s[q] & 0xC0u) != 0x80u) {
            const int l = utf8_len_valid(s, n, q);
            return l > 0 && i < q + (size_t)l;
        }
    }
    return false;
}

constexpr int kValidateBytes = 16;

__device__ __forceinline__ void validate_unit(const uint8_t* __restrict__ s, size_t n, size_t t, size_t u1,
                                              unsigned long long* __restrict__ err_pos, unsigned* __restrict__ has_cr) {
    const size_t lo = t * kValidateBytes;
    if (t >= u1 || lo >= n) return;
    bool cr = false;
    if (lo + kValidateBytes <= n && (((uintptr_t)(s + lo)) & 15) == 0) {
        const uint4 v = *reinterpret_cast<const uint4*>(s + lo);
        const uint32_t w[4] = {v.x, v.y, v.z, v.w};
        uint32_t hi_bits = 0, cr_bits = 0;
#pragma unroll
        for (int k = 0; k < 4; ++k) {
            hi_bits |= w[k] & 0x80808080u;
            const uint32_t x = w[k] ^ 0x0D0D0D0Du;
            cr_bits |= (x - 0x01010101u) & ~x & 0x80808080u;
        }
        if (cr_bits) atomicOr(has_cr, 1u);
        const int lane = threadIdx.x & 63;
        uint32_t prev = __shfl_up(w[3], 1), next = __shfl_down(w[0], 1);
        if (!hi_bits) return;
        if (lane == 0) prev = lo >= 4 ? *reinterpret_cast<const uint32_t*>(s + lo - 4) : 0u;
        if (lane == 63 || t + 1 >= u1 || lo + 2 * kValidateBytes > n) {
            next = 0;
            for (int k = 0; k < 4 && lo + kValidateBytes + k < n; ++k) next |= (uint32_t)s[lo + kValidateBytes + k] << (8 * k);
        }
        uint8_t b[24];
#pragma unroll
        for (int k = 0; k < 4; ++k) {
            b[k] = (uint8_t)(prev >> (8 * k));
            b[20 + k] = (uint8_t)(next >> (8 * k));
        }
#pragma unroll
        for (int k = 0; k < 16; ++k) b[4 + k] = (uint8_t)(w[k >> 2] >> (8 * (k & 3)));
        auto avail = [&](int x) -> size_t { const size_t i = lo + (size_t)x - 4; return i < n ? n - i : 0; };
        auto len_valid = [&](int x) -> int {
            const uint32_t b0 = b[x];
            uint32_t need, lo8 = 0x80, hi8 = 0xBF;
            if (b0 < 0x80u) return 1;
            if (b0 >= 0xC2u && b0 <= 0xDFu) need = 2;
            else if (b0 == 0xE0u) { need = 3; lo8 = 0xA0; }
            else if (b0 >= 0xE1u && b0 <= 0xECu) need = 3;
            else if (b0 == 0xEDu) { need = 3; hi8 = 0x9F; }
            else if (b0 >= 0xEEu && b0 <= 0xEFu) need = 3;
            else if (b0 == 0xF0u) { need = 4; lo8 = 0x90; }
            else if (b0 >= 0xF1u && b0 <= 0xF3u) need = 4;
            else if (b0 == 0xF4u) { need = 4; hi8 = 0x8F; }
            else return 0;
            if (avail(x) < need) return 0;
            const uint32_t b1 = b[x + 1];
            if (b1 < lo8 || b1 > hi8) return 0;
            if (need >= 3 && (b[x + 2] & 0xC0u) != 0x80u) return 0;
            if (need == 4 && (b[x + 3] & 0xC0u) != 0x80u) return 0;
            return (int)need;
        };
        int bad_k = -1;
#pragma unroll
        for (int k = 0; k < kValidateBytes; ++k) {
            const int x = 4 + k;
            if (bad_k >= 0 || b[x] < 0x80u) continue;
            bool ok;
            if ((b[x] & 0xC0u) != 0x80u) {
                ok = len_valid(x) > 0;
            } else {
                ok = false;
                bool found = false;
#pragma unroll
                for (int d = 1; d <= 3; ++d) {
                    if (found || lo + (size_t)k < (size_t)d) continue;
                    if ((b[x - d] & 0xC0u) != 0x80u) {
                        found = true;
                        const int l = len_valid(x - d);
                        ok = l > 0 && d < l;
                    }
                }
            }
            if (!ok) bad_k = k;
        }
        if (bad_k >= 0) atomicMin(err_pos, (unsigned long long)(lo + (size_t)bad_k));
        return;
    }
    const size_t hi = lo + kValidateBytes < n ? lo + kValidateBytes : n;
    for (size_t i = lo; i < hi; ++i) {
        if (s[i] == 0x0D) cr = true;
        if (!byte_ok(s, n, i)) {
            atomicMin(err_pos, (unsigned long long)i);
            break;
        }
    }
    if (cr) atomicOr(has_cr, 1u);
}

__global__ void k_validate(const uint8_t* __restrict__ s, size_t n, size_t u0, size_t u1,
                           unsigned long long* __restrict__ err_pos, unsigned* __restrict__ has_cr) {
    for (size_t b0 = u0 + (size_t)blockIdx.x * blockDim.x; b0 < u1; b0 += (size_t)gridDim.x * blockDim.x)
        validate_unit(s, n, b0 + threadIdx.x, u1, err_pos, has_cr);
}

__global__ void k_newline_map(const uint8_t* __restrict__ s, size_t n, uint8_t* __restrict__ out,
                              uint8_t* __restrict__ keep) {
    for (size_t i = (size_t)blockIdx.x * blockDim.x + threadIdx.x; i < n; i += (size_t)gridDim.x * blockDim.x) {
        const uint8_t b = s[i];
        out[i] = (b == 0x0D) ? 0x0A : b;
        keep[i] = !(b == 0x0D && i + 1 < n && s[i + 1] == 0x0A);
    }
}

const uint8_t* prepare_text(const uint8_t* d_in, size_t n, DevBuf<uint8_t>& scratch,
                            size_t* n_out, hipStream_t stream) {
    *n_out = n;
    if (n == 0) return d_in;
    DevBuf<unsigned long long> flags(2);
    const unsigned long long h_init[2] = {~0ULL, 0ULL};
    to_device(flags.p, h_init, sizeof(h_init), stream);
// ... 440 lines not shown
```

### transformer-lm_amd/csrc/train.hip

```cpp
#include <hip/hip_ext.h>

#include <algorithm>
#include <chrono>
#include <climits>
#include <cstdio>
#include <cstdlib>
#include <cstring>
#include <set>
#include <unordered_map>

#include "internal.h"
#include "prims.h"
#include "train_state.h"
#include "train_round.h"
#include "train_select.h"
#include "train_merge.h"
#include "train_apply.h"
#include "train_setup.h"

namespace bpe {

namespace {

double ms_since(std::chrono::steady_clock::time_point t0) {
    return std::chrono::duration<double, std::milli>(std::chrono::steady_clock::now() - t0).count();
}

template <class TokT>
struct HostWords {
    DevBuf<TokT> slot[kNumCls];
    DevBuf<unsigned long long> cnt[kNumCls];
    unsigned n[kNumCls] = {0, 0, 0, 0};
    DevBuf<TokT> ltok;
    DevBuf<unsigned long long> lbeg, lcnt;
    DevBuf<uint32_t> llen;
    unsigned ln = 0;
    unsigned total() const { return n[0] + n[1] + n[2] + n[3] + ln; }
    WordsDev<TokT> dev() const {
        WordsDev<TokT> W{};
        for (int c = 0; c < kNumCls; ++c) W.c[c] = SlotCls<TokT>{slot[c].p, cnt[c].p, n[c], 0, 0, 0};
        W.ltok = ltok.p; W.lbeg = lbeg.p; W.llen = llen.p; W.lcnt = lcnt.p; W.ln = ln;
        return W;
    }
};

template <class TokT>
class MergeLoop {
   public:
    MergeLoop(hipStream_t stream, Comm* comm, const uint8_t* text, int n_rounds, TrainOutput& out)
        : s_(stream), comm_(comm), text_(text), n_rounds_(n_rounds), out_(out) {}
    ~MergeLoop() {
        if (snap_st_) (void)hipHostFree(snap_st_);
        if (snap_ti_) (void)hipHostFree(snap_ti_);
        for (auto e : blk_ev_)
            if (e) (void)hipEventDestroy(e);
    }
    MergeLoop(const MergeLoop&) = delete;
    MergeLoop& operator=(const MergeLoop&) = delete;

    void build_words(const WordCounts& wc, const std::vector<std::string>& specials);
    void run();

   private:
    static constexpr int kBatch = 64;
    static constexpr int kTrips = 8;
    static_assert(2 * kTrips <= kBatch, "two blocks' timing events fit the event pool");
    static constexpr int kArgBlocks = 64;
    static constexpr unsigned kCScanBlocks = 64;
    unsigned nparts_ = 0;
    static constexpr int kTimingStride = 8;
    static constexpr unsigned long long kTarget = 4096;
    static constexpr size_t kPairLoadDiv = 2;

    void alloc_pairs(size_t cap);
    void grow_pairs();
    void ensure_pool(unsigned need);
    void push_state() { BPE_HIP(hipMemcpyAsync(st_.p, &hs_, sizeof(hs_), hipMemcpyHostToDevice, s_)); }
    void pull_state() {
        BPE_HIP(hipMemcpyAsync(&hs_, st_.p, sizeof(hs_), hipMemcpyDeviceToHost, s_));
        BPE_HIP(hipStreamSynchronize(s_));
    }
    int rebuild();
    void exhaustion();
    void compact();
    void layout_blocks();
    void build_index();
    PairsDev pairs() const { return PairsDev{pkey_.p, pcnt_.p, pflag_.p, pcap_ - 1, C_.p}; }
    ToksDev toks() const {
        return ToksDev{pool_.p, toff_.p, tlen_.p, thash_.p, tpw_.p, tkey8_.p, tmap_.p,
                       (uint32_t)(tmap_.n - 1)};
    }

    hipStream_t s_;
    Comm* comm_;
    bool sharded() const {
        static const bool force = std::getenv("BPE355_FORCE_COMM") != nullptr;
        return comm_ && (comm_->nranks > 1 || force);
    }
    const uint8_t* text_;
    int n_rounds_;
    TrainOutput& out_;

    RoundState hs_{};
    DevBuf<RoundState> st_;
    unsigned n_words_ = 0, max_len_ = 0;
    HostWords<TokT> words_;
    WordsDev<TokT> wdev_{};
    WordsDev<TokT> wdev_trip_{};
    unsigned trip_grid_ = 1;
    unsigned merge_grid_ = 1;
    double scan_bytes_ = 0, long_bytes_ = 0;
    unsigned long long long_tokens_ = 0;
    unsigned n_live_ = 0;
    DevBuf<unsigned long long> hist_;
    size_t pcap_ = 0;
    DevBuf<unsigned long long> pkey_;
    DevBuf<long long> pcnt_;
    DevBuf<unsigned> pflag_;
    DevBuf<uint4> C_;
    unsigned tok_cap_ = 0;
    size_t lr_member_ = 0;
    DevBuf<unsigned> tb_, tbc_;
    CellMarks cm_{};
    DevBuf<uint8_t> pool_;
    DevBuf<uint32_t> toff_, tlen_;
    DevBuf<unsigned long long> tmap_;
    DevBuf<unsigned long long> thash_, tpw_, tkey8_;
    DevBuf<unsigned long long> LR_;
    DevBuf<Partial> part_;
    DevBuf<uint32_t> m_a_, m_b_, m_new_, m_mode_;
    bool batched_ = false;
    bool fused_ = false;
    int max_batch_ = kMaxBatch;
    long long trips_launched_ = 0, trips_run_ = 0, rounds_batched_ = 0;
    std::unique_ptr<std::vector<int>> trip_log_;
    DevBuf<BatchState> bs_;
    DevBuf<Batch> batch_;
    DevBuf<unsigned long long> dbg_, sig_;
    DevBuf<uint32_t> tags_;
    DevBuf<int> trip_info_;
    RoundState* snap_st_ = nullptr;
    int* snap_ti_ = nullptr;
    RoundState* snap_st_dev_ = nullptr;
    int* snap_ti_dev_ = nullptr;
    hipEvent_t blk_ev_[2] = {nullptr, nullptr};
    long long slot_base_[2] = {0, 0};
    void launch_block(int slot, bool timing, std::vector<hipEvent_t>& ev);
    void finish_block(int slot, bool timing, std::vector<hipEvent_t>& ev, double& k1_ms, double& k1_bytes,
                      long long& k1_launches);
    DevBuf<unsigned long long> probe_;
    void report_probe();
    DevBuf<Partial> list_;
    static constexpr unsigned kApplyBatchBlocks = kApplyGrid;
    void reset_tags();

    DevBuf<long long> m_cnt_;
    DevBuf<RebuildStats> rs_;
    DevBuf<uint32_t> ilist_, ibeg_, ilen_;
    DevBuf<uint32_t> ix_cnt_, ix_pos_, ix_keys_, ix_vals_, ix_keys2_;
    DevBuf<uint8_t> ix_tmp_;
    HostWords<TokT> spare_;
    unsigned cls_cap_[kNumCls] = {};
    bool cls_cap_set_ = false;
    DevBuf<MoveCounts> move_counts_;
    DevBuf<unsigned> move_blk_;
    IndexDev idev_{};
    int next_index_round_ = 256;
};

template <class TokT>
void MergeLoop<TokT>::build_words(const WordCounts& wc, const std::vector<std::string>& specials) {
    std::string spb;
    std::vector<uint32_t> spo, spl;
    for (const auto& s : specials) { spo.push_back((uint32_t)spb.size()); spl.push_back((uint32_t)s.size()); spb += s; }
    DevBuf<uint8_t> d_spb(std::max<size_t>(spb.size(), 1));
    DevBuf<uint32_t> d_spo(std::max<size_t>(spo.size(), 1)), d_spl(std::max<size_t>(spl.size(), 1));
    if (!spb.empty()) BPE_HIP(hipMemcpyAsync(d_spb.p, spb.data(), spb.size(), hipMemcpyHostToDevice, s_));
    if (!spo.empty()) {
        BPE_HIP(hipMemcpyAsync(d_spo.p, spo.data(), spo.size() * 4, hipMemcpyHostToDevice, s_));
        BPE_HIP(hipMemcpyAsync(d_spl.p, spl.data(), spl.size() * 4, hipMemcpyHostToDevice, s_));
    }
    DevBuf<unsigned> cnts(2);
    BPE_HIP(hipMemsetAsync(cnts.p, 0, 8, s_));
    DevBuf<unsigned long long> w_off(wc.cap), w_cnt(wc.cap);
    DevBuf<uint32_t> w_len(wc.cap);
    hipLaunchKernelGGL(k_collect_words, dim3(ceil_div(wc.cap, (size_t)kCollectThreads * kCollectPer)),
                       dim3(kCollectThreads), 0, s_, wc.kv.p,
                       wc.pos.p, wc.cap, text_, d_spb.p, d_spo.p, d_spl.p, (int)specials.size(),
                       w_off.p, w_len.p, w_cnt.p, cnts.p, cnts.p + 1);
    BPE_HIP(hipGetLastError());
    unsigned h2[2];
    BPE_HIP(hipMemcpyAsync(h2, cnts.p, 8, hipMemcpyDeviceToHost, s_));
    BPE_HIP(hipStreamSynchronize(s_));
    n_words_ = h2[0];
    max_len_ = h2[1];
    const unsigned n = n_words_;
    hist_.alloc((size_t)kHistReplicas * 65536);
    BPE_HIP(hipMemsetAsync(hist_.p, 0, hist_.bytes(), s_));
    HostWords<TokT>& H = words_;
    unsigned long long total_tok = 0;
    H.ln = n;
    H.llen.alloc(std::max(n, 1u));
    H.lbeg.alloc(std::max(n, 1u));
    H.lcnt.alloc(std::max(n, 1u));
    if (n) {
        DevBuf<unsigned long long> len64(n);
        hipLaunchKernelGGL(k_len_u64, dim3(ceil_div(n, 256)), dim3(256), 0, s_, w_len.p, n, len64.p);
        exclusive_sum(len64.p, H.lbeg.p, n, s_);
        unsigned long long last[2];
        BPE_HIP(hipMemcpyAsync(&last[0], H.lbeg.p + n - 1, 8, hipMemcpyDeviceToHost, s_));
        BPE_HIP(hipMemcpyAsync(&last[1], len64.p + n - 1, 8, hipMemcpyDeviceToHost, s_));
        BPE_HIP(hipStreamSynchronize(s_));
        total_tok = last[0] + last[1];
    }
    H.ltok.alloc(std::max<unsigned long long>(total_tok, 1));
    if (n) {
        BPE_HIP(hipMemcpyAsync(H.llen.p, w_len.p, n * 4ull, hipMemcpyDeviceToDevice, s_));
        BPE_HIP(hipMemcpyAsync(H.lcnt.p, w_cnt.p, n * 8ull, hipMemcpyDeviceToDevice, s_));
        hipLaunchKernelGGL(k_fill_words<TokT>, dim3(ceil_div(n, 256)), dim3(256), 0, s_, text_, w_off.p,
                           w_len.p, H.lbeg.p, n, H.ltok.p);
        hipLaunchKernelGGL(k_hist_words, dim3(ceil_div(n, 256)), dim3(256), 0, s_, w_off.p,
                           w_len.p, w_cnt.p, text_, n, hist_.p);
        BPE_HIP(hipGetLastError());
    }
    hipLaunchKernelGGL(k_hist_reduce, dim3(256), dim3(256), 0, s_, hist_.p);
    out_.stats.n_words = n;
    out_.stats.n_word_tokens = (int64_t)total_tok;
    BPE_HIP(hipStreamSynchronize(s_));
    n_live_ = n;
    compact();
}

template <class TokT>
void MergeLoop<TokT>::compact() {
    HostWords<TokT>& H = words_;
    const unsigned total = H.total();
    DevBuf<MoveCounts>& mc = move_counts_;
    DevBuf<unsigned>& blk = move_blk_;
    mc.reserve(1);
    blk.reserve((size_t)kMoveBlocks * kMoveK);
    BPE_HIP(hipMemsetAsync(mc.p, 0, sizeof(MoveCounts), s_));
    const WordsDev<TokT> src = H.dev();
    if (total) {
        hipLaunchKernelGGL(k_move_count<TokT>, dim3(kMoveBlocks), dim3(256), 0, s_, src, total, blk.p, mc.p);
        hipLaunchKernelGGL(k_move_scan, dim3(1), dim3(kMoveBlocks), 0, s_, blk.p, mc.p);
    }
    MoveCounts h{};
    BPE_HIP(hipMemcpyAsync(&h, mc.p, sizeof(h), hipMemcpyDeviceToHost, s_));
    BPE_HIP(hipStreamSynchronize(s_));
    HostWords<TokT> D = std::move(spare_);
    if (!cls_cap_set_) {
        unsigned ge = h.n[kNumCls];
        for (int c = kNumCls - 1; c >= 0; --c) cls_cap_[c] = ge += h.n[c];
        cls_cap_set_ = true;
    }
    for (int c = 0; c < kNumCls; ++c) {
        D.n[c] = h.n[c];
        const size_t cap = std::max(cls_cap_[c], h.n[c]);
        D.slot[c].reserve(std::max<size_t>(cap * slot_w(c), 1));
        D.cnt[c].reserve(std::max<size_t>(cap, 1));
    }
    D.ln = h.n[kNumCls];
    D.ltok.reserve(std::max<unsigned long long>(h.long_tokens, 1));
    D.lbeg.reserve(std::max(D.ln, 1u));
    D.llen.reserve(std::max(D.ln, 1u));
    D.lcnt.reserve(std::max(D.ln, 1u));
    if (total)
        hipLaunchKernelGGL(k_move<TokT>, dim3(kMoveBlocks), dim3(256), 0, s_, src, total, D.dev(), blk.p, mc.p);
    BPE_HIP(hipGetLastError());
    BPE_HIP(hipStreamSynchronize(s_));
    spare_ = std::move(words_);
    words_ = std::move(D);
    long_tokens_ = h.long_tokens;
    n_live_ = words_.total();
    hs_.n_single = 0;
    layout_blocks();
}

template <class TokT>
void MergeLoop<TokT>::build_index() {
    const unsigned n = wdev_.off[kNumCls];
    const unsigned tcap = 256u + (unsigned)n_rounds_ + 1u;
    if (!ibeg_.p) {
        ibeg_.alloc(tcap);
        ilen_.alloc(tcap);
    }
    BPE_HIP(hipMemsetAsync(ibeg_.p, 0, ibeg_.bytes(), s_));
    BPE_HIP(hipMemsetAsync(ilen_.p, 0, ilen_.bytes(), s_));
    unsigned long long E = 0;
    DevBuf<uint32_t>&cnt = ix_cnt_, &pos = ix_pos_, &keys = ix_keys_, &vals = ix_vals_, &keys2 = ix_keys2_;
    DevBuf<uint8_t>& tmp = ix_tmp_;
    cnt.reserve(std::max(n, 1u));
    pos.reserve(std::max(n, 1u));
// ... 71 lines not shown
    long_bytes_ = (double)W.ln * 4 + (double)long_tokens_ * sizeof(TokT);
    scan_bytes_ += long_bytes_;
}

template <class TokT>
void MergeLoop<TokT>::alloc_pairs(size_t cap) {
    pcap_ = cap;
    pkey_.alloc(cap);
    pcnt_.alloc(cap);
    pflag_.alloc(cap);
    C_.alloc(cap);
    BPE_HIP(hipMemsetAsync(pkey_.p, 0, pkey_.bytes(), s_));
    BPE_HIP(hipMemsetAsync(pcnt_.p, 0, pcnt_.bytes(), s_));
    BPE_HIP(hipMemsetAsync(pflag_.p, 0, pflag_.bytes(), s_));
    hs_.capC = (unsigned)cap;
}

template <class TokT>
void MergeLoop<TokT>::grow_pairs() {
    DevBuf<unsigned long long> okey = std::move(pkey_);
    DevBuf<long long> ocnt = std::move(pcnt_);
    DevBuf<unsigned> oflag = std::move(pflag_);
    const size_t ocap = pcap_;
    alloc_pairs(ocap * 2);
    hs_.pair_used = 0;
    push_state();
    hipLaunchKernelGGL(k_rehash, dim3(ceil_div(ocap, 256)), dim3(256), 0, s_, okey.p, ocnt.p,
                       oflag.p, ocap, pairs(), st_.p);
    BPE_HIP(hipGetLastError());
    pull_state();
}

template <class TokT>
void MergeLoop<TokT>::ensure_pool(unsigned need) {
    if (hs_.pool_used + (unsigned long long)need <= hs_.pool_cap) return;
    unsigned long long cap = hs_.pool_cap;
    while (hs_.pool_used + (unsigned long long)need > cap) cap *= 2;
    BPE_REQUIRE(cap < (1ULL << 32), BPE_E_LIMIT, "token byte pool exceeds 4 GiB");
    DevBuf<uint8_t> np(cap);
    BPE_HIP(hipMemcpyAsync(np.p, pool_.p, hs_.pool_used, hipMemcpyDeviceToDevice, s_));
    pool_ = std::move(np);
    hs_.pool_cap = (unsigned)cap;
    push_state();
}

template <class TokT>
int MergeLoop<TokT>::rebuild() {
    out_.stats.n_rebuilds++;
    const int grid = 1024;
    BPE_HIP(hipMemsetAsync(rs_.p, 0, sizeof(RebuildStats), s_));
    hipLaunchKernelGGL(k_rebuild_hist, dim3(grid), dim3(256), 0, s_, pairs(), pcap_, rs_.p);
    BPE_HIP(hipGetLastError());
    RebuildStats h;
    BPE_HIP(hipMemcpyAsync(&h, rs_.p, sizeof(h), hipMemcpyDeviceToHost, s_));
    BPE_HIP(hipStreamSynchronize(s_));
    int top = -1;
    for (int k = 63; k >= 0; --k)
        if (h.bins[k]) { top = k; break; }
    if (top < 0) return h.ghosts ? 1 : 2;
    unsigned long long cum = 0;
    int k = top;
    for (; k >= 0; --k) {
        if (cum + h.bins[k] > kTarget) break;
        cum += h.bins[k];
    }
    long long T;
    if (k < 0) {
        T = 1;
    } else {
        const long long lo = 1LL << k, hi = lo << 1;
        const long long width = std::max(1LL, lo / 1024);
        hipLaunchKernelGGL(k_rebuild_sub, dim3(grid), dim3(256), 0, s_, pairs(), pcap_, lo, hi, width, rs_.p);
        BPE_HIP(hipGetLastError());
        BPE_HIP(hipMemcpyAsync(h.sub, rs_.p->sub, sizeof(h.sub), hipMemcpyDeviceToHost, s_));
        BPE_HIP(hipStreamSynchronize(s_));
        T = hi;
        for (int j = 1023; j >= 0; --j) {
            if (!h.sub[j]) continue;
            if (cum + h.sub[j] > kTarget && cum > 0) break;
            cum += h.sub[j];
            T = lo + (long long)j * width;
            if (cum > kTarget) break;
        }
    }
    hs_.T = T;
    hs_.nC = 0;
    hs_.halt = HALT_NONE;
    push_state();
    hipLaunchKernelGGL(k_build_C, dim3(grid), dim3(256), 0, s_, pairs(), pcap_, T, st_.p);
    if (batched_) {
        BPE_HIP(hipMemsetAsync(&bs_.p->list_n[0], 0, sizeof(bs_.p->list_n), s_));
        hipLaunchKernelGGL(k_apply_batch, dim3(kApplyBatchBlocks), dim3(kApplyBatchThreads), 0, s_, st_.p, bs_.p,
                           (const Batch*)batch_.p, pairs(), toks(), LR_.p, lr_member_,
                           (size_t)kMaxBatch * lr_member_, tok_cap_, part_.p, list_.p, 1, cm_, 0);
    }
    else
        hipLaunchKernelGGL(k_argmax, dim3(kArgBlocks), dim3(256), 0, s_, st_.p, pairs(), toks(), part_.p);
    nparts_ = kArgBlocks;
    BPE_HIP(hipGetLastError());
    pull_state();
    BPE_REQUIRE(!(hs_.err & ERR_C_FULL), BPE_E_NOMEM, "candidate list overflow");
    hs_.c_limit = (unsigned)std::min<unsigned long long>(
        std::max<unsigned long long>(4ull * hs_.nC, 4 * kTarget), hs_.capC);
    push_state();
    return 0;
}

constexpr double kIndexGrowth = 2.5;

template <class TokT>
void MergeLoop<TokT>::run() {
    st_.alloc(1);
    rs_.alloc(1);
    tok_cap_ = 256u + (unsigned)n_rounds_ + 1u;
    part_.alloc(std::max<size_t>(std::max<size_t>(kArgBlocks, kApplyBatchBlocks),
                                 ceil_div(4ull * tok_cap_, 256) + kCScanBlocks));
    {
        const char* e = std::getenv("BPE355_BATCH");
        max_batch_ = e ? std::min(std::atoi(e), kMaxBatch) : kMaxBatch;
        batched_ = !sharded() && max_batch_ >= 1;
    }
    lr_member_ = (2ull * tok_cap_ + 63) / 64 * 64;
    LR_.alloc(2 * (batched_ ? (size_t)kMaxBatch : 1) * lr_member_);
    BPE_HIP(hipMemsetAsync(LR_.p, 0, LR_.bytes(), s_));
    if (batched_) {
        const unsigned dense_tok = [] {
            const char* e = std::getenv("BPE355_DENSE_TOK");
            const unsigned v = e ? (unsigned)std::max(0, std::atoi(e)) : 2048u;
            return std::max(kDenseTokMin, v / 32 * 32);
        }();
        const unsigned tbw = ceil_div(tok_cap_, 1024u);
        const bool marks = tbw <= kTBMax && !(std::getenv("BPE355_CELL_MARKS") && std::getenv("BPE355_CELL_MARKS")[0] == '0');
        const unsigned sparse_from = [&] {
            const char* e = std::getenv("BPE355_SPARSE_FROM");
            return std::max(dense_tok, e ? (unsigned)std::max(0, std::atoi(e)) : 16384u);
        }();
        cm_ = CellMarks{nullptr, nullptr, marks ? tbw : 0u, dense_tok, sparse_from, nullptr};
        if (marks) {
            tb_.alloc(2ull * kTBRep * kMaxBatch * tbw);
            tbc_.alloc((size_t)kMaxBatch * tbw);
            BPE_HIP(hipMemsetAsync(tb_.p, 0, tb_.bytes(), s_));
            BPE_HIP(hipMemsetAsync(tbc_.p, 0, tbc_.bytes(), s_));
            cm_.tb = tb_.p;
            cm_.tbc = tbc_.p;
        }
    }
    if (batched_) {
        bs_.alloc(1);
        BPE_HIP(hipMemsetAsync(bs_.p, 0, sizeof(BatchState), s_));
        batch_.alloc(1);
        BPE_HIP(hipMemsetAsync(batch_.p, 0, sizeof(Batch), s_));
        trip_info_.alloc(2 * kTI * kTrips);
        if (!snap_st_) {
            BPE_HIP(hipHostMalloc(reinterpret_cast<void**>(&snap_st_), 2 * sizeof(RoundState), hipHostMallocCoherent));
            BPE_HIP(hipHostMalloc(reinterpret_cast<void**>(&snap_ti_), 2 * kTI * kTrips * sizeof(int),
                                  hipHostMallocCoherent));
            BPE_HIP(hipHostGetDevicePointer(reinterpret_cast<void**>(&snap_st_dev_), snap_st_, 0));
            BPE_HIP(hipHostGetDevicePointer(reinterpret_cast<void**>(&snap_ti_dev_), snap_ti_, 0));
            for (auto& e : blk_ev_) BPE_HIP(hipEventCreateWithFlags(&e, hipEventDisableTiming));
        }
        list_.alloc(2 * kListCap);
        const char* fe = std::getenv("BPE355_FOLD");
        fused_ = fe && fe[0] == '1';
    }
    if (batched_ && std::getenv("BPE355_CHECK_MARKS")) {
        dbg_.alloc(8);
        BPE_HIP(hipMemsetAsync(dbg_.p, 0, dbg_.bytes(), s_));
        sig_.alloc(1 + kApplyBatchBlocks);
        BPE_HIP(hipMemsetAsync(sig_.p, 0, sig_.bytes(), s_));
        cm_.sig = sig_.p;
    }
    const char* trip_log_path = std::getenv("BPE355_TRIP_LOG");
    if (batched_ && trip_log_path) trip_log_.reset(new std::vector<int>());
    m_a_.alloc(n_rounds_); m_b_.alloc(n_rounds_); m_new_.alloc(n_rounds_); m_mode_.alloc(n_rounds_);
    const char* round_log = std::getenv("BPE355_ROUND_LOG");
    if (round_log) m_cnt_.alloc(n_rounds_);
    toff_.alloc(tok_cap_); tlen_.alloc(tok_cap_);
    thash_.alloc(tok_cap_); tpw_.alloc(tok_cap_); tkey8_.alloc(tok_cap_);
    tmap_.alloc(next_pow2(16ull * tok_cap_));
    BPE_HIP(hipMemsetAsync(tmap_.p, 0, tmap_.bytes(), s_));
    const unsigned pool_cap = std::max(1u << 16, 64u * std::max(max_len_, 8u));
    pool_.alloc(pool_cap);

    if (sharded()) {
        comm_->allreduce_i64(reinterpret_cast<int64_t*>(hist_.p), 65536, s_);
        std::vector<int64_t> ml(comm_->nranks, 0);
        ml[comm_->rank] = max_len_;
        DevBuf<int64_t> d_ml(ml.size());
        BPE_HIP(hipMemcpyAsync(d_ml.p, ml.data(), ml.size() * 8, hipMemcpyHostToDevice, s_));
        comm_->allreduce_i64(d_ml.p, ml.size(), s_);
        BPE_HIP(hipMemcpyAsync(ml.data(), d_ml.p, ml.size() * 8, hipMemcpyDeviceToHost, s_));
        BPE_HIP(hipStreamSynchronize(s_));
        for (int64_t v : ml) max_len_ = std::max<unsigned>(max_len_, (unsigned)v);
    }
    int pair_log2 = 22;
    while (pair_log2 < 26 && (1ull << pair_log2) < 2ull * n_words_) ++pair_log2;
    if (const char* e = std::getenv("BPE355_PAIR_CAP_LOG2")) pair_log2 = std::max(18, std::min(30, std::atoi(e)));
    alloc_pairs(size_t(1) << pair_log2);
    const unsigned n_single_keep = hs_.n_single;
    memset(&hs_, 0, sizeof(hs_));
    hs_.n_single = n_single_keep;
    hs_.n_rounds = n_rounds_;
    hs_.ntok = 256;
    hs_.capC = (unsigned)pcap_;
    hs_.c_limit = (unsigned)pcap_;
    hs_.pool_used = 256;
    hs_.pool_cap = pool_cap;
    push_state();
    hipLaunchKernelGGL(k_init_tokens, dim3(1), dim3(256), 0, s_, toks());
    hipLaunchKernelGGL(k_init_pairs, dim3(256), dim3(256), 0, s_, hist_.p, pairs(), st_.p);
    BPE_HIP(hipGetLastError());
    pull_state();
    build_index();
    if (batched_) reset_tags();
    hs_.halt = HALT_REBUILD;
    hs_.max_len = std::max(max_len_, 1u);
    hs_.max_batch = max_batch_;
    {
        const char* e = std::getenv("BPE355_LDS_CELLS");
        hs_.narrow_limit = !(e && e[0] == '0') ? (1ll << 32) : 0;
    }
    if (batched_ && std::getenv("BPE355_PROBE") && !BPE355_PROBE_CODE)
        std::fprintf(stderr, "[bpe355 probe] BPE355_PROBE needs a library built with -DBPE355_PROBE_CODE=1 "
                             "(tools/build_variant.sh): no stamps in this one\n");
    if (batched_ && std::getenv("BPE355_PROBE") && BPE355_PROBE_CODE) {
        probe_.alloc((size_t)kProbeSlots * (n_rounds_ / kProbeTrip + 2));
        BPE_HIP(hipMemsetAsync(probe_.p, 0, probe_.bytes(), s_));
        hs_.probe = probe_.p;
    }

    const bool timing = timing_enabled();
    std::vector<hipEvent_t> ev;
    std::vector<uint32_t> hmode;
    if (timing) {
        ev.resize(2 * kBatch);
        for (auto& e : ev) BPE_HIP(hipEventCreate(&e));
    }
    double k1_ms = 0, k1_bytes = 0;
    long long k1_launches = 0;
    const bool sharded = this->sharded();

    const bool trace = std::getenv("BPE355_TRACE") != nullptr;
    const int rank = comm_ ? comm_->rank : 0;
    double h_ms[4] = {0, 0, 0, 0};
    auto now = [] { return std::chrono::steady_clock::now(); };
    auto since = [](std::chrono::steady_clock::time_point t) {
        return std::chrono::duration<double, std::milli>(std::chrono::steady_clock::now() - t).count();
    };
    for (;;) {
        if (trace)
            std::fprintf(stderr, "[bpe355 r%d] round %d halt %d nC %u T %lld pairs %llu err %u\n", rank,
                         hs_.round, hs_.halt, hs_.nC, hs_.T, hs_.pair_used, hs_.err);
        if (hs_.round >= n_rounds_) break;
        if (hs_.halt == HALT_REBUILD) {
            const auto t0 = now();
            const int r = rebuild();
            h_ms[0] += since(t0);
            if (r == 1) { exhaustion(); break; }
            if (r == 2) break;
        }
        if (batched_) {
            if (hs_.pair_used + 4ull * (hs_.ntok + kMaxBatch) * kMaxBatch > pcap_ / kPairLoadDiv) {
                const auto t0 = now();
                grow_pairs();
                h_ms[1] += since(t0);
                hs_.halt = HALT_REBUILD;
                continue;
            }
            ensure_pool((unsigned)(4 * kMaxBatch) * std::max(max_len_, 1u));
            if (hs_.halt == HALT_HOST) hs_.halt = HALT_NONE;
            hs_.host_round = next_index_round_;
            hs_.single_limit = n_live_ / 4 + 1024;
            hs_.pair_limit = pcap_ / kPairLoadDiv;
            push_state();
            const auto tb0 = now();
            {
                int slot = 0;
                launch_block(slot, timing, ev);
                for (;;) {
                    launch_block(slot ^ 1, timing, ev);
                    finish_block(slot, timing, ev, k1_ms, k1_bytes, k1_launches);
                    if (hs_.halt != HALT_NONE || hs_.err) break;
                    slot ^= 1;
                }
                finish_block(slot ^ 1, timing, ev, k1_ms, k1_bytes, k1_launches);
            }
            h_ms[3] += since(tb0);
            BPE_REQUIRE(!(hs_.err & ERR_PAIRS_FULL), BPE_E_NOMEM, "pair table overflow");
            BPE_REQUIRE(!(hs_.err & ERR_C_FULL), BPE_E_NOMEM, "candidate list overflow");
            BPE_REQUIRE(!(hs_.err & ERR_POOL), BPE_E_NOMEM, "token pool overflow");
            if (hs_.halt == HALT_DONE) break;
            if (hs_.n_single > n_live_ / 4 + 1024 || hs_.round >= next_index_round_) {
                const auto t0 = now();
                compact();
                build_index();
                reset_tags();
                push_state();
                h_ms[2] += since(t0);
                next_index_round_ = std::max(hs_.round + 512, (int)(hs_.round * kIndexGrowth));
            }
            continue;
        }
        int R = std::min(kBatch, n_rounds_ - hs_.round);
        const unsigned long long per_round = 2ull * (hs_.ntok + R + 1);
        while (hs_.pair_used + per_round * R > pcap_ / 2) {
            if (R > 8) { R /= 2; continue; }
            grow_pairs();
            hs_.halt = HALT_REBUILD;
            break;
        }
        if (hs_.halt == HALT_REBUILD) continue;
        ensure_pool((unsigned)R * std::max(max_len_, 1u));
        const long long start_round = hs_.round;
        for (int k = 0; k < R; ++k) {
            const bool timed = timing && (start_round + k) % kTimingStride == 0;
            const long long rnd = start_round + k;
            unsigned long long* LRc = LR_.p + (size_t)(rnd & 1) * 2 * tok_cap_;
            unsigned long long* LRo = LR_.p + (size_t)((rnd + 1) & 1) * 2 * tok_cap_;
            hipExtLaunchKernelGGL(k_merge<TokT>, dim3(merge_grid_), dim3(256), 0, s_,
                                  timed ? ev[2 * k] : nullptr, timed ? ev[2 * k + 1] : nullptr, 0,
                                  st_.p, (const Partial*)part_.p, (int)nparts_, pairs(), toks(),
                                  wdev_, idev_, LRc, m_a_.p, m_b_.p, m_new_.p, m_mode_.p, m_cnt_.p);
            if (sharded) {
                const size_t ntok_bound = 256 + (size_t)rnd + 1;
                comm_->allreduce_i64(reinterpret_cast<int64_t*>(LRc), 2 * ntok_bound, s_);
            }
            const unsigned ntb = 256u + (unsigned)rnd + 1u;
            const unsigned cell_blocks = ceil_div(4ull * ntb, kApplyThreads);
            const unsigned c_blocks = std::min<unsigned>(kCScanBlocks,
                                                         std::max(1u, ceil_div(hs_.c_limit, kApplyThreads)));
            hipLaunchKernelGGL(k_apply_argmax, dim3(cell_blocks + c_blocks), dim3(kApplyThreads), 0, s_, st_.p,
                               pairs(), toks(), (const unsigned long long*)LRc, LRo, ntb, cell_blocks,
                               part_.p);
            nparts_ = cell_blocks + c_blocks;
        }
        BPE_HIP(hipGetLastError());
        pull_state();
        if (timing) {
            const int done = (int)(hs_.round - start_round);
            hmode.resize(std::max(done, 1));
            if (done)
                BPE_HIP(hipMemcpy(hmode.data(), m_mode_.p + start_round, done * 4ull, hipMemcpyDeviceToHost));
            const double slot_avg = scan_bytes_ / std::max(1u, idev_.n_slot_words + words_.ln);
            for (int k = 0; k < std::min(done, R); ++k) {
                if ((start_round + k) % kTimingStride) continue;
                float t = 0;
                BPE_HIP(hipEventElapsedTime(&t, ev[2 * k], ev[2 * k + 1]));
                k1_ms += t;
                k1_bytes += hmode[k] == 0xffffffffu ? scan_bytes_
                                                    : hmode[k] * (4.0 + slot_avg) + long_bytes_;
                ++k1_launches;
            }
        }
        BPE_REQUIRE(!(hs_.err & ERR_PAIRS_FULL), BPE_E_NOMEM, "pair table overflow");
        BPE_REQUIRE(!(hs_.err & ERR_C_FULL), BPE_E_NOMEM, "candidate list overflow");
        BPE_REQUIRE(!(hs_.err & ERR_POOL), BPE_E_NOMEM, "token pool overflow");
        if (hs_.halt == HALT_DONE) break;
        if (hs_.n_single > n_live_ / 4 + 1024 || hs_.round >= next_index_round_) {
            compact();
            build_index();
            push_state();
            next_index_round_ = std::max(hs_.round + 512, (int)(hs_.round * 2.5));
        }
    }
    for (auto& e : ev) (void)hipEventDestroy(e);
    if (trace)
        std::fprintf(stderr, "[bpe355] merge loop host clock: rebuild %.1f ms, grow %.1f, compact+index %.1f, trip blocks %.1f\n",
                     h_ms[0], h_ms[1], h_ms[2], h_ms[3]);
    if (round_log && hs_.round) {
        const int rd = hs_.round;
        std::vector<uint32_t> va(rd), vb(rd), vn(rd), vm(rd);
        std::vector<long long> vc(rd);
        BPE_HIP(hipMemcpy(va.data(), m_a_.p, rd * 4ull, hipMemcpyDeviceToHost));
        BPE_HIP(hipMemcpy(vb.data(), m_b_.p, rd * 4ull, hipMemcpyDeviceToHost));
        BPE_HIP(hipMemcpy(vn.data(), m_new_.p, rd * 4ull, hipMemcpyDeviceToHost));
        BPE_HIP(hipMemcpy(vm.data(), m_mode_.p, rd * 4ull, hipMemcpyDeviceToHost));
        BPE_HIP(hipMemcpy(vc.data(), m_cnt_.p, rd * 8ull, hipMemcpyDeviceToHost));
        if (FILE* f = std::fopen(round_log, "wb")) {
            for (int r = 0; r < rd; ++r) {
                std::fwrite(&va[r], 4, 1, f); std::fwrite(&vb[r], 4, 1, f); std::fwrite(&vn[r], 4, 1, f);
                std::fwrite(&vm[r], 4, 1, f); std::fwrite(&vc[r], 8, 1, f);
            }
            std::fclose(f);
        }
    }
    if (dbg_.p) {
        unsigned long long d[8];
        BPE_HIP(hipMemcpy(d, dbg_.p, sizeof(d), hipMemcpyDeviceToHost));
        std::fprintf(stderr, "[bpe355 check-marks] nonzero cells left after the clear: %llu (first: trip %llu member %llu "
                             "cell %llu); bitmap words left: %llu; apply workgroups with another view: %llu (first: "
                             "trip %llu workgroup %llu)\n", d[0], d[1], d[2], d[3], d[4], d[5], d[6], d[7]);
        BPE_REQUIRE(d[0] == 0 && d[4] == 0 && d[5] == 0, BPE_E_HIP,
                    "cell marks: a delta outside the marked blocks, or apply workgroups that listed different blocks");
    }
    if (trip_log_ && !trip_log_->empty()) {
        if (FILE* f = std::fopen(trip_log_path, "wb")) {
            std::fwrite(trip_log_->data(), sizeof(int), trip_log_->size(), f);
            std::fclose(f);
        }
    }
    if (probe_.p) report_probe();
    if (batched_) {
        BatchState b{};
        BPE_HIP(hipMemcpy(&b, bs_.p, sizeof(b), hipMemcpyDeviceToHost));
        out_.stats.n_trips = trips_run_;
        out_.stats.n_rounds_batched = rounds_batched_;
        if (BPE355_STATS_CODE && std::getenv("BPE355_TRACE")) {
            std::fprintf(stderr, "[bpe355] trips: list overflow %llu, head miss %llu, short %llu; k:", b.n_overflow,
                         b.n_headmiss, b.n_short);
            for (int i = 0; i <= kMaxBatch; ++i) std::fprintf(stderr, " %llu", b.k_hist[i]);
            std::fprintf(stderr, "; k=1 because: a==b %llu, not fresh %llu, no list %llu, P2 fails %llu, tie %llu\n",
                         b.k1_why[0], b.k1_why[1], b.k1_why[2], b.k1_why[3], b.k1_why[4]);
            std::fprintf(stderr, "[bpe355] batch ended by: cap %llu, list ran out %llu, candidate k failed the token "
                         "rules %llu, count gap / tie %llu, P1 alone %llu\n", b.end_why[0], b.end_why[1],
                         b.end_why[2], b.end_why[3], b.end_why[4]);
        }
    }
    out_.stats.merge_kernel_ms = k1_ms;
    out_.stats.merge_kernel_launches = k1_launches;
    out_.stats.merge_kernel_bytes = k1_bytes;
    out_.stats.n_pairs_final = (int64_t)hs_.pair_used;
    out_.stats.n_rounds_device = hs_.round;

    const int rd = hs_.round;
    std::vector<uint32_t> ma(rd), mb(rd), mn(rd);
    if (rd) {
        BPE_HIP(hipMemcpyAsync(ma.data(), m_a_.p, rd * 4ull, hipMemcpyDeviceToHost, s_));
        BPE_HIP(hipMemcpyAsync(mb.data(), m_b_.p, rd * 4ull, hipMemcpyDeviceToHost, s_));
        BPE_HIP(hipMemcpyAsync(mn.data(), m_new_.p, rd * 4ull, hipMemcpyDeviceToHost, s_));
        BPE_HIP(hipStreamSynchronize(s_));
    }
    std::vector<std::pair<std::string, std::string>> tail = std::move(out_.merges);
    out_.merges.clear();
    auto& tb = out_.tok_bytes;
    tb.clear();
    for (int b = 0; b < 256; ++b) tb.push_back(std::string(1, (char)b));
    for (int r = 0; r < rd; ++r) {
        std::string nb = tb[ma[r]] + tb[mb[r]];
        if (mn[r] == tb.size()) tb.push_back(nb);
        else BPE_REQUIRE(mn[r] < tb.size() && tb[mn[r]] == nb, BPE_E_HIP,
                         "device token dedupe disagrees with host replay");
        out_.merges.emplace_back(tb[ma[r]], tb[mb[r]]);
    }
    for (auto& m : tail) out_.merges.push_back(std::move(m));
}

template <class TokT>
void MergeLoop<TokT>::report_probe() {
    std::vector<unsigned long long> pr(probe_.n);
    BPE_HIP(hipMemcpy(pr.data(), probe_.p, probe_.bytes(), hipMemcpyDeviceToHost));
    const char* names[] = {"sel:issue", "sel:p1+list+meta", "sel:rule", "sel:fill", "gap sel>merge", "merge:pop",
                           "merge:rewrite", "merge:flush", "gap merge>apply", "apply:clear", "apply:items",
                           "apply:blocktop", "apply:end", "gap apply>sel"};
    const int from[] = {0, 1, 2, 3, 4, 5, 6, 7, 8, 9, 10, 11, 12, 13};
    const int to[] = {1, 2, 3, 4, 5, 6, 7, 8, 9, 10, 11, 12, 13, 16};
    double acc[14] = {};
    int n = 0;
    double tails[4] = {};
    int nt4 = 0;
    for (size_t t = 0; t + 1 < pr.size() / kProbeSlots; ++t) {
        const unsigned long long* p = &pr[kProbeSlots * t];
        bool ok = true;
        for (int i = 0; i < 14; ++i) ok &= p[i] != 0;
        if (!ok) continue;
        for (int i = 0; i < 13; ++i) acc[i] += (double)(p[to[i]] - p[from[i]]) * 0.01;
        ++n;
        if (p[14] && p[15] && p[16]) {
            tails[0] += (double)(long long)(p[14] - p[8]) * 0.01;
            tails[1] += (double)(long long)(p[9] - p[14]) * 0.01;
            tails[2] += (double)(long long)(p[15] - p[13]) * 0.01;
            tails[3] += (double)(long long)(p[16] - p[15]) * 0.01;
            ++nt4;
        }
    }
    std::fprintf(stderr, "[bpe355 probe] %d sampled trips, mean us:", n);
    for (int i = 0; i < 13 && n; ++i) std::fprintf(stderr, " %s %.2f |", names[i], acc[i] / n);
    std::fprintf(stderr, "\n");
    {
        double r[4] = {};
        int nr = 0;
        for (size_t t = 0; t + 1 < pr.size() / kProbeSlots; ++t) {
            const unsigned long long* p = &pr[kProbeSlots * t];
            if (!(p[2] && p[17] && p[18] && p[19] && p[3])) continue;
            r[0] += (double)(p[17] - p[2]) * 0.01; r[1] += (double)(p[18] - p[17]) * 0.01;
            r[2] += (double)(p[19] - p[18]) * 0.01; r[3] += (double)(p[3] - p[19]) * 0.01;
            ++nr;
        }
        if (nr)
            std::fprintf(stderr, "[bpe355 probe] select rule: p1 %.2f | head+meta %.2f | clash+k+gap %.2f | record %.2f\n",
                         r[0] / nr, r[1] / nr, r[2] / nr, r[3] / nr);
        double q[6] = {};
        int nq = 0;
        for (size_t t = 0; t + 1 < pr.size() / kProbeSlots; ++t) {
            const unsigned long long* p = &pr[kProbeSlots * t];
            if (!p[1] || !p[24] || !p[25] || !p[26] || !p[27] || !p[28] || !p[2]) continue;
            q[0] += (double)((long long)p[24] - (long long)p[1]) * 0.01; q[1] += (double)((long long)p[25] - (long long)p[24]) * 0.01;
            q[2] += (double)((long long)p[26] - (long long)p[1]) * 0.01; q[3] += (double)((long long)p[27] - (long long)p[25]) * 0.01;
            q[4] += (double)((long long)p[28] - (long long)p[27]) * 0.01; q[5] += (double)((long long)p[2] - (long long)p[28]) * 0.01;
            ++nq;
        }
        if (nq)
            std::fprintf(stderr, "[bpe355 probe] select phase 1 (list thread 0): list entry %.2f | metadata+dedupe %.2f | "
                                 "(wave 0 partials %.2f) | barrier %.2f | rank %.2f | minima+barrier %.2f (%d trips)\n",
                         q[0] / nq, q[1] / nq, q[2] / nq, q[3] / nq, q[4] / nq, q[5] / nq, nq);
        std::vector<double> nls, rl;
        for (size_t t = 0; t + 1 < pr.size() / kProbeSlots; ++t) {
            const unsigned long long* p = &pr[kProbeSlots * t];
            if (p[30]) nls.push_back((double)p[30] - 1);
            if (p[27] && p[29]) rl.push_back(((long long)p[29] - (long long)p[27]) * 0.01);
        }
        {
            double a = 0, b = 0, c = 0;
            int n = 0;
            for (size_t t = 0; t + 1 < pr.size() / kProbeSlots; ++t) {
                const unsigned long long* p = &pr[kProbeSlots * t];
                if (!p[27] || !p[29] || !p[31] || !p[28]) continue;
                a += ((long long)p[29] - (long long)p[27]) * 0.01;
// ... 74 lines not shown
    tags_.reserve(std::max(idev_.n_slot_words, 1u));
    BPE_HIP(hipMemsetAsync(tags_.p, 0, std::max(idev_.n_slot_words, 1u) * sizeof(uint32_t), s_));
}

template <class TokT>
void MergeLoop<TokT>::launch_block(int slot, bool timing, std::vector<hipEvent_t>& ev) {
    const size_t lr_member = lr_member_, lr_parity = (size_t)kMaxBatch * lr_member;
    const unsigned ntb = tok_cap_;
    const unsigned apply_blocks = kApplyBatchBlocks;
    const int sparse_hint = cm_.tbw && (long long)hs_.ntok + 2ll * kTrips * kMaxBatch >= (long long)cm_.sparse_from;
    int* ti = trip_info_.p + (size_t)slot * kTI * kTrips;
    slot_base_[slot] = trips_launched_;
    for (int t = 0; t < kTrips; ++t) {
        const bool timed = timing && (trips_launched_ + t) % kTimingStride == 0;
        hipEvent_t* e = &ev[2 * ((size_t)slot * kTrips + t)];
        const SelOut so{m_a_.p, m_b_.p, m_new_.p, m_mode_.p, m_cnt_.p, ti, t};
        if (fused_ && sizeof(TokT) == 2) {
            hipExtLaunchKernelGGL(k_trip<TokT>, dim3(trip_grid_), dim3(kTripThreads), 0, s_,
                                  timed ? e[0] : nullptr, timed ? e[1] : nullptr, 0,
                                  st_.p, bs_.p, pairs(), toks(), wdev_trip_, idev_, batch_.p, (const Partial*)part_.p,
                                  (const Partial*)list_.p, so, LR_.p, lr_member, lr_parity, tags_.p, cm_);
        } else {
            hipLaunchKernelGGL(k_select, dim3(1), dim3(kSelThreads), 0, s_, (const RoundState*)st_.p, bs_.p, toks(),
                               idev_, batch_.p, (const Partial*)part_.p, (const Partial*)list_.p, so);
            hipExtLaunchKernelGGL(k_merge_batch<TokT>, dim3(merge_grid_), dim3(256), 0, s_,
                                  timed ? e[0] : nullptr, timed ? e[1] : nullptr, 0,
                                  st_.p, (const Batch*)batch_.p, pairs(), toks(), wdev_, idev_, LR_.p, lr_member,
                                  lr_parity, tags_.p, cm_);
        }
        if (dbg_.p)
            hipLaunchKernelGGL(k_check_clear, dim3(256), dim3(256), 0, s_, (const Batch*)batch_.p, (const unsigned long long*)LR_.p,
                               lr_member, lr_parity, (const unsigned*)cm_.tb, cm_.tbw, dbg_.p);
        hipLaunchKernelGGL(k_apply_batch, dim3(apply_blocks), dim3(kApplyBatchThreads), 0, s_, st_.p, bs_.p,
                           (const Batch*)batch_.p, pairs(), toks(), LR_.p, lr_member, lr_parity, ntb, part_.p,
                           list_.p, 0, cm_, sparse_hint);
        if (sig_.p)
            hipLaunchKernelGGL(k_check_sig, dim3(1), dim3(256), 0, s_, (const Batch*)batch_.p, sig_.p,
                               (unsigned)kApplyBatchBlocks, dbg_.p);
    }
    static_assert(sizeof(RoundState) % 4 == 0, "k_snapshot copies words");
    hipLaunchKernelGGL(k_snapshot, dim3(1), dim3(256), 0, s_, (const uint32_t*)st_.p,
                       (unsigned)(sizeof(RoundState) / 4), (const uint32_t*)ti, (unsigned)(kTI * kTrips),
                       (uint32_t*)(snap_st_dev_ + slot), (uint32_t*)(snap_ti_dev_ + (size_t)slot * kTI * kTrips));
    BPE_HIP(hipGetLastError());
    BPE_HIP(hipEventRecord(blk_ev_[slot], s_));
    trips_launched_ += kTrips;
}

template <class TokT>
void MergeLoop<TokT>::finish_block(int slot, bool timing, std::vector<hipEvent_t>& ev, double& k1_ms,
                                   double& k1_bytes, long long& k1_launches) {
    BPE_HIP(hipEventSynchronize(blk_ev_[slot]));
    hs_ = snap_st_[slot];
    const int* ti = snap_ti_ + (size_t)slot * kTI * kTrips;
    for (int t = 0; t < kTrips; ++t) {
        trips_run_ += ti[kTI * t + 1] > 0;
        rounds_batched_ += ti[kTI * t + 1] > 1 ? ti[kTI * t + 1] : 0;
        if (trip_log_) trip_log_->insert(trip_log_->end(), ti + kTI * t, ti + kTI * (t + 1));
    }
    if (!timing) return;
    const double slot_avg = scan_bytes_ / std::max(1u, idev_.n_slot_words + words_.ln);
    for (int t = 0; t < kTrips; ++t) {
        if ((slot_base_[slot] + t) % kTimingStride || ti[kTI * t + 1] <= 0) continue;
        float ms = 0;
        const hipEvent_t* e = &ev[2 * ((size_t)slot * kTrips + t)];
        BPE_HIP(hipEventElapsedTime(&ms, e[0], e[1]));
        const bool full = ti[kTI * t + 2] != 0;
        k1_ms += ms;
        k1_bytes += full ? scan_bytes_ : long_bytes_ + (double)(unsigned)ti[kTI * t + 3] * (4.0 + slot_avg);
        ++k1_launches;
    }
}

template <class TokT>
void MergeLoop<TokT>::exhaustion() {
    const int rd = hs_.round;
    std::vector<uint32_t> ma(rd), mb(rd), mn(rd);
    if (rd) {
        BPE_HIP(hipMemcpyAsync(ma.data(), m_a_.p, rd * 4ull, hipMemcpyDeviceToHost, s_));
        BPE_HIP(hipMemcpyAsync(mb.data(), m_b_.p, rd * 4ull, hipMemcpyDeviceToHost, s_));
        BPE_HIP(hipMemcpyAsync(mn.data(), m_new_.p, rd * 4ull, hipMemcpyDeviceToHost, s_));
    }
    DevBuf<unsigned long long> keys(std::max<size_t>(hs_.pair_used, 1));
    DevBuf<unsigned> nk(1);
    BPE_HIP(hipMemsetAsync(nk.p, 0, 4, s_));
    hipLaunchKernelGGL(k_collect_present, dim3(1024), dim3(256), 0, s_, pairs(), pcap_, keys.p, nk.p);
    unsigned hk = 0;
    BPE_HIP(hipMemcpyAsync(&hk, nk.p, 4, hipMemcpyDeviceToHost, s_));
    BPE_HIP(hipStreamSynchronize(s_));
    std::vector<unsigned long long> hkeys(hk);
    if (hk) {
        BPE_HIP(hipMemcpyAsync(hkeys.data(), keys.p, hk * 8ull, hipMemcpyDeviceToHost, s_));
        BPE_HIP(hipStreamSynchronize(s_));
    }
    std::vector<std::string> tb;
    for (int b = 0; b < 256; ++b) tb.push_back(std::string(1, (char)b));
    for (int r = 0; r < rd; ++r) {
        std::string nb = tb[ma[r]] + tb[mb[r]];
        if (mn[r] == tb.size()) tb.push_back(nb);
        else BPE_REQUIRE(mn[r] < tb.size() && tb[mn[r]] == nb, BPE_E_HIP,
                         "device token dedupe disagrees with host replay");
    }
    std::vector<std::pair<std::string, std::string>> ghosts;
    ghosts.reserve(hk);
    for (auto k : hkeys) ghosts.emplace_back(tb[k >> 32], tb[k & 0xffffffffu]);
    std::sort(ghosts.begin(), ghosts.end(), [](const auto& x, const auto& y) { return x > y; });
    const size_t left = (size_t)(n_rounds_ - rd);
    if (ghosts.size() > left) ghosts.resize(left);
    out_.stats.n_rounds_host = (int64_t)ghosts.size();
    out_.merges = std::move(ghosts);
}

}

namespace {

void agree_on_errors(Comm* comm, const Error* mine, hipStream_t stream) {
    const int R = comm->nranks;
    std::vector<int64_t> v(3 * (size_t)R, 0);
    if (mine) {
        v[3 * comm->rank] = mine->code;
        v[3 * comm->rank + 1] = mine->sys_errno;
        const size_t p = mine->msg.find("position ");
        v[3 * comm->rank + 2] = p == std::string::npos ? 0 : std::stoll(mine->msg.substr(p + 9));
    }
    DevBuf<int64_t> d(v.size());
    BPE_HIP(hipMemcpyAsync(d.p, v.data(), v.size() * 8, hipMemcpyHostToDevice, stream));
    comm->allreduce_i64(d.p, v.size(), stream);
    BPE_HIP(hipMemcpyAsync(v.data(), d.p, v.size() * 8, hipMemcpyDeviceToHost, stream));
    BPE_HIP(hipStreamSynchronize(stream));
    for (int r = 0; r < R; ++r) {
        const int code = (int)v[3 * r];
        if (!code) continue;
        if (r == comm->rank && mine) throw *mine;
        if (code == BPE_E_UTF8)
            throw Error{code, "'utf-8' codec can't decode byte at position " + std::to_string(v[3 * r + 2])};
        throw Error{code, "rank " + std::to_string(r) + " failed before training (code " + std::to_string(code) + ")",
                    (int)v[3 * r + 1]};
    }
}

}

bool per_round_exchange() {
    const char* ex = std::getenv("BPE355_EXCHANGE");
    return ex && std::string(ex) == "rounds";
}

void train_on_device(const uint8_t* d_raw, size_t n, int vocab_size,
                     const std::vector<std::string>& specials, Comm* comm, hipStream_t stream,
                     TrainOutput& out, const TrainOpts& opt, Prepared* pre) {
    const auto t0 = std::chrono::steady_clock::now();
    out = TrainOutput{};
    DevBuf<uint8_t> scratch;
    size_t tn = 0;
    const uint8_t* text = nullptr;
    const bool several = comm && comm->nranks > 1;
    WordCounts wc;
    float count_ms = 0;
    std::chrono::steady_clock::time_point t1;
    {
        Error err{0, ""};
        bool failed = opt.has_pending;
        if (failed) err = opt.pending;
        if (!failed && pre) {
            text = pre->text;
            tn = pre->n;
            wc = std::move(pre->wc);
            count_ms = pre->count_kernel_ms;
            out.stats.t_prepare_ms = pre->t_prepare_ms;
            out.stats.n_bytes = (int64_t)tn;
            t1 = std::chrono::steady_clock::now() - std::chrono::duration_cast<std::chrono::steady_clock::duration>(
                                                         std::chrono::duration<double, std::milli>(pre->t_count_ms));
        } else if (!failed) {
            try {
                text = prepare_text(d_raw, n, scratch, &tn, stream);
                out.stats.t_prepare_ms = ms_since(t0);
                out.stats.n_bytes = (int64_t)tn;
                t1 = std::chrono::steady_clock::now();
                count_words(text, tn, wc, stream, timing_enabled() ? &count_ms : nullptr);
            } catch (const Error& e) {
                if (!several && !opt.slab_offset) throw;
                err = e;
                failed = true;
            }
        }
        if (failed && err.code == BPE_E_UTF8 && opt.slab_offset) {
            const size_t p = err.msg.find("position ");
            if (p != std::string::npos)
                err.msg = "'utf-8' codec can't decode byte at position " +
                          std::to_string(std::stoull(err.msg.substr(p + 9)) + opt.slab_offset);
        }
        if (several) agree_on_errors(comm, failed ? &err : nullptr, stream);
        else if (failed) throw err;
    }

    const long long rounds = merge_rounds(vocab_size, specials);

    out.stats.t_count_ms = ms_since(t1);
    out.stats.count_kernel_ms = count_ms;
    out.stats.count_kernel_bytes = (double)tn;
    out.stats.n_pretokens = (int64_t)wc.n_pretokens;
    out.stats.n_count_records = (int64_t)wc.n_records;
    out.stats.count_reduce_ms = wc.reduce_ms;
    out.stats.count_partial_ms = wc.partial_ms;
    out.stats.n_count_batches = (int64_t)wc.batches;
    if (rounds <= 0) {
        out.stats.t_total_ms = ms_since(t0);
        return;
    }
    BPE_REQUIRE(rounds < (1LL << 31) - 512, BPE_E_LIMIT, "vocab_size too large");
    DevBuf<uint8_t> union_text;
    Comm* loop_comm = comm;
    const bool per_round = per_round_exchange();
    if (comm && !per_round && (comm->nranks > 1 || std::getenv("BPE355_FORCE_EXCHANGE"))) {
        auto te = std::chrono::steady_clock::now();
        uint64_t uw = 0;
        union_word_tables(text, wc, comm, stream, union_text, &uw, &out.stats);
        text = union_text.p;
        loop_comm = nullptr;
        out.stats.t_exchange_ms = ms_since(te);
        out.stats.n_exchanged_words = (int64_t)uw;
    }
    if (!opt.merge_loop) {
        out.stats.t_total_ms = ms_since(t0);
        return;
    }
    train_words(text, wc, vocab_size, specials, stream, out, loop_comm, &wc);
    out.stats.t_total_ms = ms_since(t0);
}

long long merge_rounds(int vocab_size, const std::vector<std::string>& specials) {
    std::set<std::string> base;
    for (const auto& s : specials) base.insert(s);
    for (int b = 0; b < 256; ++b) base.insert(std::string(1, (char)b));
    return (long long)vocab_size - (long long)base.size();
}

void train_words(const uint8_t* text, const WordCounts& wc, int vocab_size, const std::vector<std::string>& specials,
                 hipStream_t stream, TrainOutput& out, Comm* loop_comm, WordCounts* drop_after_build) {
    const long long rounds = merge_rounds(vocab_size, specials);
    if (rounds <= 0) return;
    BPE_REQUIRE(rounds < (1LL << 31) - 512, BPE_E_LIMIT, "vocab_size too large");
    auto go = [&](auto tag) {
        using TokT = decltype(tag);
        auto t2 = std::chrono::steady_clock::now();
        MergeLoop<TokT> loop(stream, loop_comm, text, (int)rounds, out);
        loop.build_words(wc, specials);
        if (drop_after_build) { WordCounts drop = std::move(*drop_after_build); }
        out.stats.t_words_ms = ms_since(t2);
        auto t3 = std::chrono::steady_clock::now();
        loop.run();
        out.stats.t_merge_ms = ms_since(t3);
    };
    if (256 + rounds + 1 < 65535) go(uint16_t{});
    else go(uint32_t{});
}

}
```

Before: 24930.

## Pool device buffers, events and pinned snapshots across training calls

Adds a size-classed device memory arena so DevBuf allocations inside train_on_device reuse freed blocks, both within a call and across calls, instead of calling hipMalloc/hipFree each time. hipEvents in ChunkTrack and the pinned host snapshot buffers of the merge loop are also pooled and reused. It additionally adds an env-gated timeline tracer that wraps HIP sync and alloc calls for profiling. The trade-off is cached device memory held between calls, which feeds into the memory-fit estimate, plus an extra memset when a block is reused.

Measured after the change: 27180 (median of 4 runs). 1.09x the previous value.

```diff
diff --git a/transformer-lm_amd/csrc/api.hip b/transformer-lm_amd/csrc/api.hip
--- a/transformer-lm_amd/csrc/api.hip
+++ b/transformer-lm_amd/csrc/api.hip
@@ -1,7 +1,9 @@
 #include <dlfcn.h>
 #include <hip/hip_version.h>
 
+#include <algorithm>
 #include <cerrno>
+#include <chrono>
 #include <cstdio>
 #include <cstdlib>
 #include <cstring>
@@ -17,8 +19,57 @@
 #include "count.h"
 #include "drive.h"
 #include "internal.h"
+#include "timeline_wrap.h"
 
 namespace bpe {
+
+namespace tl {
+std::atomic<bool> g_active{false};
+namespace {
+struct Rec {
+    const char* what;
+    const char* file;
+    int line;
+    double start, dur;
+};
+std::mutex g_m;
+std::vector<Rec> g_recs;
+std::chrono::steady_clock::time_point g_t0;
+}
+double now_ms() { return std::chrono::duration<double, std::milli>(std::chrono::steady_clock::now() - g_t0).count(); }
+void note(const char* what, const char* file, int line, double start_ms, double dur_ms) {
+    std::lock_guard<std::mutex> g(g_m);
+    g_recs.push_back(Rec{what, file, line, start_ms, dur_ms});
+}
+Call::Call(const char* n) : name(n) {
+    if (!std::getenv("BPE355_STEP_TIMELINE")) return;
+    std::lock_guard<std::mutex> g(g_m);
+    if (g_active.load()) return;
+    g_recs.clear();
+    g_t0 = std::chrono::steady_clock::now();
+    g_active = owner = true;
+}
+Call::~Call() {
+    if (!owner) return;
+    const double end = now_ms();
+    std::vector<Rec> recs;
+    {
+        std::lock_guard<std::mutex> g(g_m);
+        g_active = false;
+        recs.swap(g_recs);
+    }
+    std::stable_sort(recs.begin(), recs.end(), [](const Rec& a, const Rec& b) { return a.start < b.start; });
+    double blocked = 0;
+    std::fprintf(stderr, "[bpe355 timeline] %s: entry at 0.000 ms\n", name);
+    for (const Rec& r : recs) {
+        std::fprintf(stderr, "[bpe355 timeline] %s:%d %s start %.3f ms dur %.3f ms\n", r.file, r.line, r.what, r.start,
+                     r.dur);
+        blocked += r.dur;
+    }
+    std::fprintf(stderr, "[bpe355 timeline] %s: return at %.3f ms, %zu lines, %.3f ms in them (threads overlap)\n", name,
+                 end, recs.size(), blocked);
+}
+}
 
 namespace {
 thread_local std::string g_err;
@@ -195,6 +246,7 @@
         BPE_REQUIRE(device < n, BPE_E_ARG, "device " + std::to_string(device) + " is not visible");
         size_t b = bpe::corpus_release(device);
         b += bpe::scratch_release(device);
+        b += bpe::arena_drain(device);
         if (freed_bytes) *freed_bytes = b;
     });
 }
@@ -212,12 +264,14 @@
 
 int bpe_train_device(const uint8_t* d_data, size_t n, int vocab_size, const char* const* specials,
                      int n_specials, bpe_comm* comm, void* hip_stream, bpe_result** out) {
+    bpe::tl::Call tl_call("bpe_train_device");
     if (n && !d_data) return bpe::guarded([] { throw bpe::Error{BPE_E_ARG, "data is NULL"}; });
     return train_common(d_data, n, vocab_size, specials, n_specials, comm, hip_stream, out);
 }
 
 int bpe_train_buffer(const uint8_t* data, size_t n, int vocab_size, const char* const* specials,
                      int n_specials, bpe_comm* comm, bpe_result** out) {
+    bpe::tl::Call tl_call("bpe_train_buffer");
     return bpe::guarded([&] {
         BPE_REQUIRE(out, BPE_E_ARG, "out is NULL");
         *out = nullptr;
@@ -236,6 +290,7 @@
 
 int bpe_train_buffer_gpus(const uint8_t* data, size_t n, int vocab_size, const char* const* specials,
                           int n_specials, int n_gpus, bpe_result** out) {
+    bpe::tl::Call tl_call("bpe_train_buffer_gpus");
     return bpe::guarded([&] {
         BPE_REQUIRE(out, BPE_E_ARG, "out is NULL");
         *out = nullptr;
@@ -253,6 +308,7 @@
 
 int bpe_train_file(const char* path, int vocab_size, const char* const* specials, int n_specials,
                    int n_gpus, bpe_result** out) {
+    bpe::tl::Call tl_call("bpe_train_file");
     return bpe::guarded([&] {
         BPE_REQUIRE(out, BPE_E_ARG, "out is NULL");
         *out = nullptr;
@@ -270,6 +326,7 @@
 
 int bpe_train_file_comm(const char* path, int vocab_size, const char* const* specials, int n_specials,
                         bpe_comm* comm, int split, bpe_result** out) {
+    bpe::tl::Call tl_call("bpe_train_file_comm");
     return bpe::guarded([&] {
         BPE_REQUIRE(out, BPE_E_ARG, "out is NULL");
         *out = nullptr;
diff --git a/transformer-lm_amd/csrc/arena.h b/transformer-lm_amd/csrc/arena.h
--- /dev/null
+++ b/transformer-lm_amd/csrc/arena.h
@@ -0,0 +1,136 @@
+#pragma once
+
+#include <cstddef>
+#include <map>
+#include <mutex>
+#include <vector>
+
+namespace bpe {
+
+inline size_t arena_class(size_t bytes) {
+    constexpr size_t kMin = 512, kLarge = (size_t)64 << 20, kStep = (size_t)2 << 20;
+    if (bytes <= kMin) return kMin;
+    if (bytes > kLarge) return (bytes + kStep - 1) / kStep * kStep;
+    size_t q = kMin;
+    while (2 * q < bytes) q *= 2;
+    const size_t step = q / 4;
+    return (bytes + step - 1) / step * step;
+}
+
+template <class Backend>
+class Arena {
+   public:
+    using Stream = typename Backend::Stream;
+    static constexpr int kOutOfMemory = -1000001;
+    using Lists = std::map<size_t, std::vector<void*>>;
+
+    struct Scope {
+        int dev = 0;
+        Stream stream{};
+        Lists free_;
+        size_t free_bytes = 0;
+    };
+
+    explicit Arena(Backend b = Backend()) : b_(b) {}
+    Backend& backend() { return b_; }
+
+    int alloc(Scope& sc, size_t bytes, void** p, size_t* cap) {
+        const size_t cls = arena_class(bytes);
+        *cap = cls;
+        *p = pop(sc.free_, cls);
+        if (*p) {
+            sc.free_bytes -= cls;
+            return b_.zero(*p, bytes, sc.stream);
+        }
+        {
+            std::lock_guard<std::mutex> g(m_);
+            auto it = cache_.find(sc.dev);
+            if (it != cache_.end() && (*p = pop(it->second.lists, cls))) it->second.bytes -= cls;
+        }
+        if (*p) return b_.zero(*p, bytes, sc.stream);
+        int rc = b_.alloc(sc.dev, p, cls);
+        if (rc == kOutOfMemory) {
+            drain(sc.dev);
+            drain_scope(sc);
+            rc = b_.alloc(sc.dev, p, cls);
+        }
+        if (rc != 0) *p = nullptr;
+        return rc;
+    }
+
+    void release(Scope& sc, void* p, size_t cap, int dev) {
+        if (dev != sc.dev) {
+            b_.free(dev, p);
+            return;
+        }
+        sc.free_[cap].push_back(p);
+        sc.free_bytes += cap;
+    }
+
+    int close(Scope& sc) {
+        const int rc = b_.sync(sc.stream);
+        std::lock_guard<std::mutex> g(m_);
+        PerDev& d = cache_[sc.dev];
+        for (auto& kv : sc.free_)
+            for (void* p : kv.second) {
+                d.lists[kv.first].push_back(p);
+                d.bytes += kv.first;
+            }
+        sc.free_.clear();
+        sc.free_bytes = 0;
+        return rc;
+    }
+
+    size_t drain(int dev) {
+        std::vector<std::pair<int, void*>> drop;
+        size_t bytes = 0;
+        {
+            std::lock_guard<std::mutex> g(m_);
+            for (auto& kd : cache_) {
+                if (dev >= 0 && kd.first != dev) continue;
+                for (auto& kv : kd.second.lists)
+                    for (void* p : kv.second) drop.emplace_back(kd.first, p);
+                bytes += kd.second.bytes;
+                kd.second.lists.clear();
+                kd.second.bytes = 0;
+            }
+        }
+        for (auto& x : drop) b_.free(x.first, x.second);
+        return bytes;
+    }
+
+    size_t drain_scope(Scope& sc) {
+        if (sc.free_.empty()) return 0;
+        (void)b_.sync(sc.stream);
+        const size_t bytes = sc.free_bytes;
+        for (auto& kv : sc.free_)
+            for (void* p : kv.second) b_.free(sc.dev, p);
+        sc.free_.clear();
+        sc.free_bytes = 0;
+        return bytes;
+    }
+
+    size_t cached_bytes(int dev) {
+        std::lock_guard<std::mutex> g(m_);
+        auto it = cache_.find(dev);
+        return it == cache_.end() ? 0 : it->second.bytes;
+    }
+
+   private:
+    struct PerDev {
+        Lists lists;
+        size_t bytes = 0;
+    };
+    static void* pop(Lists& l, size_t cls) {
+        auto it = l.find(cls);
+        if (it == l.end() || it->second.empty()) return nullptr;
+        void* p = it->second.back();
+        it->second.pop_back();
+        return p;
+    }
+    Backend b_;
+    std::mutex m_;
+    std::map<int, PerDev> cache_;
+};
+
+}
diff --git a/transformer-lm_amd/csrc/arena.hip b/transformer-lm_amd/csrc/arena.hip
--- /dev/null
+++ b/transformer-lm_amd/csrc/arena.hip
@@ -0,0 +1,87 @@
+#include <memory>
+
+#include "arena.h"
+#include "bpe_common.h"
+
+namespace bpe {
+
+namespace {
+
+struct HipBackend {
+    using Stream = hipStream_t;
+    int alloc(int, void** p, size_t bytes) {
+        const hipError_t e =
+            tl::timed("hipMalloc", __FILE__, __LINE__, [&] { return hipMalloc(p, bytes); });
+        if (e == hipErrorOutOfMemory) {
+            (void)hipGetLastError();
+            return Arena<HipBackend>::kOutOfMemory;
+        }
+        return (int)e;
+    }
+    void free(int dev, void* p) {
+        int cur = dev;
+        (void)hipGetDevice(&cur);
+        if (cur != dev) (void)hipSetDevice(dev);
+        (void)tl::timed("hipFree", __FILE__, __LINE__, [&] { return hipFree(p); });
+        if (cur != dev) (void)hipSetDevice(cur);
+    }
+    int sync(hipStream_t s) {
+        return (int)tl::timed("hipStreamSynchronize", __FILE__, __LINE__, [&] { return hipStreamSynchronize(s); });
+    }
+    int zero(void* p, size_t bytes, hipStream_t s) { return (int)hipMemsetAsync(p, 0, bytes, s); }
+};
+
+using HipArena = Arena<HipBackend>;
+HipArena& arena() {
+    static HipArena* a = new HipArena;
+    return *a;
+}
+thread_local HipArena::Scope* t_scope = nullptr;
+
+}
+
+ArenaScope::ArenaScope(hipStream_t stream) {
+    if (t_scope) return;
+    auto sc = std::make_unique<HipArena::Scope>();
+    BPE_HIP(hipGetDevice(&sc->dev));
+    sc->stream = stream;
+    t_scope = sc.release();
+    owner_ = true;
+}
+
+ArenaScope::~ArenaScope() {
+    if (!owner_) return;
+    std::unique_ptr<HipArena::Scope> sc(t_scope);
+    t_scope = nullptr;
+    (void)arena().close(*sc);
+}
+
+bool arena_alloc(size_t bytes, void** p, size_t* cap, int* dev) {
+    HipArena::Scope* sc = t_scope;
+    if (!sc) return false;
+    const int rc = arena().alloc(*sc, bytes, p, cap);
+    if (rc == HipArena::kOutOfMemory)
+        throw Error{BPE_E_NOMEM, "device allocation of " + std::to_string(bytes) + " bytes failed (out of memory)"};
+    if (rc != 0) {
+        if (*p) arena().release(*sc, *p, *cap, sc->dev);
+        *p = nullptr;
+        throw Error{BPE_E_HIP, std::string("device allocation: ") + hipGetErrorString((hipError_t)rc)};
+    }
+    *dev = sc->dev;
+    return true;
+}
+
+void arena_release(void* p, size_t cap, int dev) {
+    if (HipArena::Scope* sc = t_scope) arena().release(*sc, p, cap, dev);
+    else arena().backend().free(dev, p);
+}
+
+size_t arena_drain(int dev) { return arena().drain(dev); }
+
+size_t arena_cached_bytes(int dev) {
+    size_t b = arena().cached_bytes(dev);
+    if (t_scope && t_scope->dev == dev) b += t_scope->free_bytes;
+    return b;
+}
+
+}
diff --git a/transformer-lm_amd/csrc/bpe_common.h b/transformer-lm_amd/csrc/bpe_common.h
--- a/transformer-lm_amd/csrc/bpe_common.h
+++ b/transformer-lm_amd/csrc/bpe_common.h
@@ -7,6 +7,7 @@
 #include <string>
 
 #include "../../include/bpe355.h"
+#include "timeline.h"
 
 namespace bpe {
 
@@ -30,6 +31,20 @@
         if (!(cond)) throw ::bpe::Error{(code), (msg)};       \
     } while (0)
 
+struct ArenaScope {
+    explicit ArenaScope(hipStream_t stream);
+    ~ArenaScope();
+    ArenaScope(const ArenaScope&) = delete;
+    ArenaScope& operator=(const ArenaScope&) = delete;
+
+   private:
+    bool owner_ = false;
+};
+bool arena_alloc(size_t bytes, void** p, size_t* cap, int* dev);
+void arena_release(void* p, size_t cap, int dev);
+size_t arena_drain(int dev);
+size_t arena_cached_bytes(int dev);
+
 template <class T>
 struct DevBuf {
     T* p = nullptr;
@@ -38,16 +53,26 @@
     explicit DevBuf(size_t count) { alloc(count); }
     DevBuf(const DevBuf&) = delete;
     DevBuf& operator=(const DevBuf&) = delete;
-    DevBuf(DevBuf&& o) noexcept : p(o.p), n(o.n) { o.p = nullptr; o.n = 0; }
+    DevBuf(DevBuf&& o) noexcept : p(o.p), n(o.n), cap_(o.cap_), dev_(o.dev_) { o.p = nullptr; o.n = 0; o.cap_ = 0; }
     DevBuf& operator=(DevBuf&& o) noexcept {
-        if (this != &o) { release(); p = o.p; n = o.n; o.p = nullptr; o.n = 0; }
+        if (this != &o) {
+            release();
+            p = o.p; n = o.n; cap_ = o.cap_; dev_ = o.dev_;
+            o.p = nullptr; o.n = 0; o.cap_ = 0;
+        }
         return *this;
     }
     ~DevBuf() { release(); }
     void alloc(size_t count) {
         release();
         if (!count) return;
-        const hipError_t e = hipMalloc(&p, count * sizeof(T));
+        void* q = nullptr;
+        if (arena_alloc(count * sizeof(T), &q, &cap_, &dev_)) {
+            p = static_cast<T*>(q);
+            n = count;
+            return;
+        }
+        const hipError_t e = tl::timed("hipMalloc", __FILE__, __LINE__, [&] { return hipMalloc(&p, count * sizeof(T)); });
         if (e == hipErrorOutOfMemory) {
             (void)hipGetLastError();
             p = nullptr;
@@ -61,11 +86,19 @@
         if (count > n || !p) alloc(count);
     }
     void release() {
-        if (p) (void)hipFree(p);
+        if (p) {
+            if (cap_) arena_release(p, cap_, dev_);
+            else (void)tl::timed("hipFree", __FILE__, __LINE__, [&] { return hipFree(p); });
+        }
         p = nullptr;
         n = 0;
+        cap_ = 0;
     }
     size_t bytes() const { return n * sizeof(T); }
+
+   private:
+    size_t cap_ = 0;
+    int dev_ = 0;
 };
 
 enum : int { CLS_OTHER = 0, CLS_LETTER = 1, CLS_NUMBER = 2, CLS_SPACE = 3 };
diff --git a/transformer-lm_amd/csrc/comm.hip b/transformer-lm_amd/csrc/comm.hip
--- a/transformer-lm_amd/csrc/comm.hip
+++ b/transformer-lm_amd/csrc/comm.hip
@@ -8,6 +8,7 @@
 #include <vector>
 
 #include "internal.h"
+#include "timeline_wrap.h"
 
 namespace bpe {
 
diff --git a/transformer-lm_amd/csrc/count.hip b/transformer-lm_amd/csrc/count.hip
--- a/transformer-lm_amd/csrc/count.hip
+++ b/transformer-lm_amd/csrc/count.hip
@@ -11,6 +11,7 @@
 #include "stage.h"
 #include "stage2.h"
 #include "tokstart.h"
+#include "timeline_wrap.h"
 
 #ifndef BPE355_COUNT_EARLY_PREFETCH
 #define BPE355_COUNT_EARLY_PREFETCH 1
@@ -792,7 +793,7 @@
     BPE_HIP(hipGetDevice(&dev));
     size_t free_b = 0, total_b = 0;
     BPE_HIP(hipMemGetInfo(&free_b, &total_b));
-    const size_t avail = free_b + scratch_cached_bytes(dev);
+    const size_t avail = free_b + scratch_cached_bytes(dev) + arena_cached_bytes(dev);
     const size_t reserve = std::max<size_t>(total_b / 16, n_bytes / 2);
     size_t fit = avail > reserve ? (avail - reserve) / (6 * sizeof(uint64_t) + 1) : 0;
     if (const char* e = std::getenv("BPE355_REC_POOL_FIT")) fit = (size_t)std::atof(e);
diff --git a/transformer-lm_amd/csrc/drive.hip b/transformer-lm_amd/csrc/drive.hip
--- a/transformer-lm_amd/csrc/drive.hip
+++ b/transformer-lm_amd/csrc/drive.hip
@@ -12,12 +12,14 @@
 #include <cstdio>
 #include <cstring>
 #include <exception>
+#include <map>
 #include <memory>
 #include <mutex>
 #include <thread>
 #include <vector>
 
 #include "drive.h"
+#include "timeline_wrap.h"
 
 namespace bpe {
 
@@ -453,12 +455,40 @@
     std::condition_variable cv;
     size_t prefix = 0;
     bool failed = false;
-    explicit ChunkTrack(size_t n) : ev(n, nullptr), ready(n, 0) {
-        for (auto& e : ev) BPE_HIP(hipEventCreateWithFlags(&e, hipEventDisableTiming));
-    }
-    ~ChunkTrack() {
+    ChunkTrack(size_t n, int device) : ev(n, nullptr), ready(n, 0), dev(device) {
+        {
+            std::lock_guard<std::mutex> g(event_pool().m);
+            auto& f = event_pool().free_[dev];
+            for (auto& e : ev) {
+                if (f.empty()) break;
+                e = f.back();
+                f.pop_back();
+            }
+        }
+        try {
+            for (auto& e : ev)
+                if (!e) BPE_HIP(hipEventCreateWithFlags(&e, hipEventDisableTiming));
+        } catch (...) {
+            give_back();
+            throw;
+        }
+    }
+    ~ChunkTrack() { give_back(); }
+    int dev;
+    struct EventPool {
+        std::mutex m;
+        std::map<int, std::vector<hipEvent_t>> free_;
+    };
+    static EventPool& event_pool() {
+        static EventPool* p = new EventPool;
+        return *p;
+    }
+    void give_back() {
+        std::lock_guard<std::mutex> g(event_pool().m);
+        auto& f = event_pool().free_[dev];
         for (auto& e : ev)
-            if (e) (void)hipEventDestroy(e);
+            if (e) f.push_back(e);
+        ev.clear();
     }
     void mark(size_t i) {
         std::lock_guard<std::mutex> g(m);
@@ -483,16 +513,21 @@
     return (size_t)(e ? std::max(1, std::atoi(e)) : 256) << 20;
 }
 
-std::vector<size_t> segment_cuts(const Source& src, size_t off, size_t len, size_t seg) {
+std::vector<size_t> segment_cuts(const Source& src, size_t off, size_t len, size_t seg, size_t* n_regular = nullptr) {
     std::vector<size_t> cut{0};
     std::vector<uint8_t> win(1u << 16);
-    for (size_t want = seg; want + seg / 2 < len; want += seg) {
+    auto cut_near = [&](size_t want) {
         const size_t lo = want - std::min(want, win.size() - 2);
         const size_t hi = want + 2;
         src.read(off + lo, hi - lo, win.data());
         const size_t p = bpe_safe_split(win.data(), hi - lo, want - lo);
         if (p > 0 && lo + p > cut.back()) cut.push_back(lo + p);
-    }
+    };
+    for (size_t want = seg; want + seg / 2 < len; want += seg) cut_near(want);
+    if (n_regular) *n_regular = cut.size();
+    const size_t last = cut.back(), rem = len - last;
+    if (rem / 8 >= win.size())
+        for (size_t part = rem / 2; part >= rem / 8; part /= 2) cut_near(last + rem - part);
     cut.push_back(len);
     return cut;
 }
@@ -502,13 +537,12 @@
 bool load_and_count(const Source& src, size_t off, size_t len, uint8_t* d_dst, int device, int threads,
                     hipStream_t stream, Prepared& pre, size_t min_cap) {
     const auto t0 = std::chrono::steady_clock::now();
-    const std::vector<size_t> cut = segment_cuts(src, off, len, segment_bytes());
     const size_t chunks = (len + kStageChunk - 1) / kStageChunk;
-    ChunkTrack track(chunks);
+    ChunkTrack track(chunks, device);
     const int t_n = (int)std::max<size_t>(1, std::min<size_t>((size_t)threads, chunks));
     std::atomic<size_t> next{0};
     std::vector<std::exception_ptr> errs(t_n);
-    DmaStreams dma(device, dma_streams());
+    const DmaStreams& dma = cached_dma(device, 0);
     auto reader = [&](int t) {
         const hipStream_t s = dma.pick(t);
         void* buf[2] = {nullptr, nullptr};
@@ -522,6 +556,7 @@
                 if (last[k] != ~(size_t)0) BPE_HIP(hipEventSynchronize(track.ev[last[k]]));
                 const size_t lo = i * kStageChunk, n = std::min(kStageChunk, len - lo);
                 src.read(off + lo, n, static_cast<uint8_t*>(buf[k]));
+                if (i == 0) BPE_TL_MARK("load: first hipMemcpyAsync");
                 BPE_HIP(hipMemcpyAsync(d_dst + lo, buf[k], n, hipMemcpyHostToDevice, s));
                 BPE_HIP(hipEventRecord(track.ev[i], s));
                 last[k] = i;
@@ -540,6 +575,16 @@
     };
     std::vector<std::thread> th;
     for (int t = 0; t < t_n; ++t) th.emplace_back(reader, t);
+    size_t n_regular = 0;
+    std::vector<size_t> cut;
+    try {
+        cut = segment_cuts(src, off, len, segment_bytes(), &n_regular);
+    } catch (...) {
+        track.fail();
+        next.store(chunks);
+        for (auto& x : th) x.join();
+        throw;
+    }
     ValidatePass vp;
     CountPass cp;
     bool ok = true;
@@ -556,19 +601,20 @@
             for (; waited < need; ++waited) BPE_HIP(hipStreamWaitEvent(stream, track.ev[waited], 0));
             vp.range(cut[k], cut[k + 1]);
             cp.range(cut[k], cut[k + 1]);
-            if (agg_every > 0 && (k + 1) % agg_every == 0 && k + 2 < cut.size()) cp.partial();
+            if (agg_every > 0 && (k + 1) % agg_every == 0 && k + 1 < n_regular) cp.partial();
         }
     } catch (...) {
         track.fail();
         next.store(chunks);
-        for (auto& x : th) x.join();
+        for (auto& x : th) BPE_TL_JOIN(x);
         throw;
     }
-    for (auto& x : th) x.join();
+    for (auto& x : th) BPE_TL_JOIN(x);
     for (auto& e : errs)
         if (e) std::rethrow_exception(e);
     BPE_REQUIRE(ok, BPE_E_IO, "corpus load failed");
     const double load_ms = std::chrono::duration<double, std::milli>(std::chrono::steady_clock::now() - t0).count();
+    BPE_TL_MARK("load: last byte enqueued, readers joined");
     unsigned long long bad = 0;
     bool cr = false;
     vp.finish(&bad, &cr);
@@ -587,6 +633,7 @@
     pre.t_prepare_ms = 0;
     pre.t_count_ms = std::chrono::duration<double, std::milli>(std::chrono::steady_clock::now() - t0).count() - load_ms;
     pre.load_ms = load_ms;
+    BPE_TL_MARK("count: done");
     return true;
 }
 
@@ -708,6 +755,43 @@
 
 bool inproc_ranks() { return std::getenv("BPE355_INPROC_RANKS") != nullptr; }
 
+namespace {
+struct StreamLease {
+    hipStream_t s = nullptr;
+    int dev = 0;
+    struct Pool {
+        std::mutex m;
+        std::map<int, std::vector<hipStream_t>> free_;
+    };
+    static Pool& pool() {
+        static Pool* p = new Pool;
+        return *p;
+    }
+    StreamLease() {
+        BPE_HIP(hipGetDevice(&dev));
+        {
+            std::lock_guard<std::mutex> g(pool().m);
+            auto& f = pool().free_[dev];
+            if (!f.empty()) {
+                s = f.back();
+                f.pop_back();
+            }
+        }
+        if (!s) BPE_HIP(hipStreamCreateWithFlags(&s, hipStreamNonBlocking));
+    }
+    ~StreamLease() {
+        if (hipStreamSynchronize(s) != hipSuccess) {
+            (void)hipStreamDestroy(s);
+            return;
+        }
+        std::lock_guard<std::mutex> g(pool().m);
+        pool().free_[dev].push_back(s);
+    }
+    StreamLease(const StreamLease&) = delete;
+    StreamLease& operator=(const StreamLease&) = delete;
+};
+}
+
 std::vector<int> pick_devices(int n_gpus) {
     int cur = 0, n = 0;
     BPE_HIP(hipGetDevice(&cur));
@@ -729,9 +813,9 @@
     if (g == 1) {
         static const bool dtrace = std::getenv("BPE355_DRIVE_TRACE") != nullptr;
         auto ms = [&] { return std::chrono::duration<double, std::milli>(std::chrono::steady_clock::now() - t0).count(); };
-        hipStream_t s = nullptr;
-        BPE_HIP(hipStreamCreateWithFlags(&s, hipStreamNonBlocking));
-        struct SGuard { hipStream_t s; ~SGuard() { (void)hipStreamDestroy(s); } } sg{s};
+        StreamLease lease;
+        const hipStream_t s = lease.s;
+        ArenaScope arena(s);
         std::unique_ptr<CorpusBuf> d = corpus_take(std::max<size_t>(src.size, 1));
         const double a_ms = ms();
         Prepared pre;
@@ -766,6 +850,7 @@
             hipStream_t s = nullptr;
             BPE_HIP(hipStreamCreateWithFlags(&s, hipStreamNonBlocking));
             struct SGuard { hipStream_t s; ~SGuard() { (void)hipStreamDestroy(s); } } sg{s};
+            ArenaScope arena(s);
             const size_t len = cut[r + 1] - cut[r];
             std::unique_ptr<CorpusBuf> dbuf = corpus_take(std::max<size_t>(len, 1));
             uint8_t* const d = dbuf->b.p;
@@ -792,7 +877,7 @@
     std::vector<std::thread> th;
     for (int r = 1; r < g; ++r) th.emplace_back(work, r);
     work(0);
-    for (auto& x : th) x.join();
+    for (auto& x : th) BPE_TL_JOIN(x);
     for (auto& e : errs)
         if (e) std::rethrow_exception(e);
     if (per_round_exchange())
@@ -822,6 +907,7 @@
     hipStream_t s = nullptr;
     BPE_HIP(hipStreamCreateWithFlags(&s, hipStreamNonBlocking));
     struct SGuard { hipStream_t s; ~SGuard() { (void)hipStreamDestroy(s); } } sg{s};
+    ArenaScope arena(s);
     std::unique_ptr<CorpusBuf> dbuf = corpus_take(std::max<size_t>(hi - lo, 1));
     uint8_t* const d = dbuf->b.p;
     TrainOpts opt;
diff --git a/transformer-lm_amd/csrc/exchange.hip b/transformer-lm_amd/csrc/exchange.hip
--- a/transformer-lm_amd/csrc/exchange.hip
+++ b/transformer-lm_amd/csrc/exchange.hip
@@ -9,6 +9,7 @@
 #include "internal.h"
 #include "prims.h"
 #include "stage.h"
+#include "timeline_wrap.h"
 
 namespace bpe {
 
diff --git a/transformer-lm_amd/csrc/hostio.hip b/transformer-lm_amd/csrc/hostio.hip
--- a/transformer-lm_amd/csrc/hostio.hip
+++ b/transformer-lm_amd/csrc/hostio.hip
@@ -2,6 +2,7 @@
 #include <cstring>
 
 #include "internal.h"
+#include "timeline_wrap.h"
 
 namespace bpe {
 namespace {
diff --git a/transformer-lm_amd/csrc/text.hip b/transformer-lm_amd/csrc/text.hip
--- a/transformer-lm_amd/csrc/text.hip
+++ b/transformer-lm_amd/csrc/text.hip
@@ -9,6 +9,7 @@
 #include "prims.h"
 #include "pretok.h"
 #include "stage.h"
+#include "timeline_wrap.h"
 
 namespace bpe {
 
diff --git a/transformer-lm_amd/csrc/timeline.h b/transformer-lm_amd/csrc/timeline.h
--- /dev/null
+++ b/transformer-lm_amd/csrc/timeline.h
@@ -0,0 +1,39 @@
+#pragma once
+
+#include <hip/hip_runtime.h>
+
+#include <atomic>
+#include <chrono>
+
+namespace bpe {
+namespace tl {
+
+extern std::atomic<bool> g_active;
+inline bool on() { return g_active.load(std::memory_order_relaxed); }
+double now_ms();
+void note(const char* what, const char* file, int line, double start_ms, double dur_ms);
+inline void mark(const char* what, const char* file, int line) {
+    if (on()) note(what, file, line, now_ms(), 0);
+}
+
+struct Call {
+    bool owner = false;
+    const char* name;
+    explicit Call(const char* name);
+    ~Call();
+};
+
+template <class F>
+inline auto timed(const char* what, const char* file, int line, F&& f) -> decltype(f()) {
+    if (!on()) return f();
+    const double a = now_ms();
+    auto r = f();
+    note(what, file, line, a, now_ms() - a);
+    return r;
+}
+
+}
+}
+
+#define BPE_TL_MARK(what) ::bpe::tl::mark(what, __FILE__, __LINE__)
+#define BPE_TL_JOIN(th) ::bpe::tl::timed("thread join", __FILE__, __LINE__, [&] { (th).join(); return 0; })
diff --git a/transformer-lm_amd/csrc/timeline_wrap.h b/transformer-lm_amd/csrc/timeline_wrap.h
--- /dev/null
+++ b/transformer-lm_amd/csrc/timeline_wrap.h
@@ -0,0 +1,18 @@
+#pragma once
+
+#include "timeline.h"
+
+#define BPE_TL_WRAP(fn, ...) ::bpe::tl::timed(#fn, __FILE__, __LINE__, [&] { return (fn)(__VA_ARGS__); })
+#define hipStreamSynchronize(...) BPE_TL_WRAP(hipStreamSynchronize, __VA_ARGS__)
+#define hipEventSynchronize(...) BPE_TL_WRAP(hipEventSynchronize, __VA_ARGS__)
+#define hipDeviceSynchronize(...) BPE_TL_WRAP(hipDeviceSynchronize, __VA_ARGS__)
+#define hipMemcpy(...) BPE_TL_WRAP(hipMemcpy, __VA_ARGS__)
+#define hipStreamCreateWithFlags(...) BPE_TL_WRAP(hipStreamCreateWithFlags, __VA_ARGS__)
+#define hipStreamCreateWithPriority(...) BPE_TL_WRAP(hipStreamCreateWithPriority, __VA_ARGS__)
+#define hipStreamDestroy(...) BPE_TL_WRAP(hipStreamDestroy, __VA_ARGS__)
+#define hipEventCreate(...) BPE_TL_WRAP(hipEventCreate, __VA_ARGS__)
+#define hipEventCreateWithFlags(...) BPE_TL_WRAP(hipEventCreateWithFlags, __VA_ARGS__)
+#define hipEventDestroy(...) BPE_TL_WRAP(hipEventDestroy, __VA_ARGS__)
+#define hipHostMalloc(...) BPE_TL_WRAP(hipHostMalloc, __VA_ARGS__)
+#define hipHostFree(...) BPE_TL_WRAP(hipHostFree, __VA_ARGS__)
+#define hipMemGetInfo(...) BPE_TL_WRAP(hipMemGetInfo, __VA_ARGS__)
diff --git a/transformer-lm_amd/csrc/train.hip b/transformer-lm_amd/csrc/train.hip
--- a/transformer-lm_amd/csrc/train.hip
+++ b/transformer-lm_amd/csrc/train.hip
@@ -6,6 +6,7 @@
 #include <cstdio>
 #include <cstdlib>
 #include <cstring>
+#include <mutex>
 #include <set>
 #include <unordered_map>
 
@@ -17,6 +18,7 @@
 #include "train_merge.h"
 #include "train_apply.h"
 #include "train_setup.h"
+#include "timeline_wrap.h"
 
 namespace bpe {
 
@@ -44,16 +46,69 @@
     }
 };
 
+struct SnapSet {
+    void* st = nullptr;
+    void* ti = nullptr;
+    void* st_dev = nullptr;
+    void* ti_dev = nullptr;
+    hipEvent_t ev[2] = {nullptr, nullptr};
+    size_t ti_bytes = 0;
+    int dev = -1;
+};
+struct SnapCache {
+    std::mutex m;
+    std::vector<SnapSet> free_;
+};
+SnapCache& snap_cache() {
+    static SnapCache* c = new SnapCache;
+    return *c;
+}
+SnapSet snap_take(size_t ti_bytes) {
+    int dev = 0;
+    BPE_HIP(hipGetDevice(&dev));
+    {
+        std::lock_guard<std::mutex> g(snap_cache().m);
+        auto& f = snap_cache().free_;
+        for (size_t i = 0; i < f.size(); ++i)
+            if (f[i].dev == dev && f[i].ti_bytes == ti_bytes) {
+                const SnapSet x = f[i];
+                f.erase(f.begin() + i);
+                return x;
+            }
+    }
+    SnapSet x;
+    x.dev = dev;
+    x.ti_bytes = ti_bytes;
+    try {
+        BPE_HIP(hipHostMalloc(&x.st, 2 * sizeof(RoundState), hipHostMallocCoherent));
+        BPE_HIP(hipHostMalloc(&x.ti, ti_bytes, hipHostMallocCoherent));
+        BPE_HIP(hipHostGetDevicePointer(&x.st_dev, x.st, 0));
+        BPE_HIP(hipHostGetDevicePointer(&x.ti_dev, x.ti, 0));
+        for (auto& e : x.ev) BPE_HIP(hipEventCreateWithFlags(&e, hipEventDisableTiming));
+    } catch (...) {
+        if (x.st) (void)hipHostFree(x.st);
+        if (x.ti) (void)hipHostFree(x.ti);
+        for (auto e : x.ev)
+            if (e) (void)hipEventDestroy(e);
+        throw;
+    }
+    return x;
+}
+void snap_give(const SnapSet& x) {
+    std::lock_guard<std::mutex> g(snap_cache().m);
+    snap_cache().free_.push_back(x);
+}
+
 template <class TokT>
 class MergeLoop {
    public:
     MergeLoop(hipStream_t stream, Comm* comm, const uint8_t* text, int n_rounds, TrainOutput& out)
         : s_(stream), comm_(comm), text_(text), n_rounds_(n_rounds), out_(out) {}
     ~MergeLoop() {
-        if (snap_st_) (void)hipHostFree(snap_st_);
-        if (snap_ti_) (void)hipHostFree(snap_ti_);
-        for (auto e : blk_ev_)
-            if (e) (void)hipEventDestroy(e);
+        if (snap_.st) {
+            (void)hipStreamSynchronize(s_);
+            snap_give(snap_);
+        }
     }
     MergeLoop(const MergeLoop&) = delete;
     MergeLoop& operator=(const MergeLoop&) = delete;
@@ -139,6 +194,7 @@
     DevBuf<unsigned long long> dbg_, sig_;
     DevBuf<uint32_t> tags_;
     DevBuf<int> trip_info_;
+    SnapSet snap_;
     RoundState* snap_st_ = nullptr;
     int* snap_ti_ = nullptr;
     RoundState* snap_st_dev_ = nullptr;
@@ -516,12 +572,13 @@
         BPE_HIP(hipMemsetAsync(batch_.p, 0, sizeof(Batch), s_));
         trip_info_.alloc(2 * kTI * kTrips);
         if (!snap_st_) {
-            BPE_HIP(hipHostMalloc(reinterpret_cast<void**>(&snap_st_), 2 * sizeof(RoundState), hipHostMallocCoherent));
-            BPE_HIP(hipHostMalloc(reinterpret_cast<void**>(&snap_ti_), 2 * kTI * kTrips * sizeof(int),
-                                  hipHostMallocCoherent));
-            BPE_HIP(hipHostGetDevicePointer(reinterpret_cast<void**>(&snap_st_dev_), snap_st_, 0));
-            BPE_HIP(hipHostGetDevicePointer(reinterpret_cast<void**>(&snap_ti_dev_), snap_ti_, 0));
-            for (auto& e : blk_ev_) BPE_HIP(hipEventCreateWithFlags(&e, hipEventDisableTiming));
+            snap_ = snap_take(2 * kTI * kTrips * sizeof(int));
+            snap_st_ = static_cast<RoundState*>(snap_.st);
+            snap_ti_ = static_cast<int*>(snap_.ti);
+            snap_st_dev_ = static_cast<RoundState*>(snap_.st_dev);
+            snap_ti_dev_ = static_cast<int*>(snap_.ti_dev);
+            blk_ev_[0] = snap_.ev[0];
+            blk_ev_[1] = snap_.ev[1];
         }
         list_.alloc(2 * kListCap);
         const char* fe = std::getenv("BPE355_FOLD");
@@ -593,6 +650,7 @@
         hs_.probe = probe_.p;
     }
 
+    BPE_TL_MARK("merge: setup done");
     const bool timing = timing_enabled();
     std::vector<hipEvent_t> ev;
     std::vector<uint32_t> hmode;
@@ -727,6 +785,7 @@
             next_index_round_ = std::max(hs_.round + 512, (int)(hs_.round * 2.5));
         }
     }
+    BPE_TL_MARK("merge: last trip done");
     for (auto& e : ev) (void)hipEventDestroy(e);
     if (trace)
         std::fprintf(stderr, "[bpe355] merge loop host clock: rebuild %.1f ms, grow %.1f, compact+index %.1f, trip blocks %.1f\n",
@@ -1107,6 +1166,7 @@
                      TrainOutput& out, const TrainOpts& opt, Prepared* pre) {
     const auto t0 = std::chrono::steady_clock::now();
     out = TrainOutput{};
+    ArenaScope arena(stream);
     DevBuf<uint8_t> scratch;
     size_t tn = 0;
     const uint8_t* text = nullptr;
@@ -1204,9 +1264,11 @@
         loop.build_words(wc, specials);
         if (drop_after_build) { WordCounts drop = std::move(*drop_after_build); }
         out.stats.t_words_ms = ms_since(t2);
+        BPE_TL_MARK("words: built");
         auto t3 = std::chrono::steady_clock::now();
         loop.run();
         out.stats.t_merge_ms = ms_since(t3);
+        BPE_TL_MARK("merge: done");
     };
     if (256 + rounds + 1 < 65535) go(uint16_t{});
     else go(uint32_t{});
```
